# zenghjian/SceneSplat

Measured on AMD Instinct MI355X. Metric: Gaussians/s encoder fwd+bwd, 102k-pt chunks, higher is better.
Workload: dtype bf16

## Files before the change

### include/scenesplat_hip.h

```cpp
#ifndef SCENESPLAT_HIP_H
#define SCENESPLAT_HIP_H
#include <stddef.h>
#include <stdint.h>

#ifdef __cplusplus
extern "C" {
#endif

struct ihipStream_t;
typedef struct ihipStream_t* ss_stream_t;

#define SS_MAX_ORDERS 8
enum { SS_ORDER_Z = 0, SS_ORDER_Z_TRANS = 1, SS_ORDER_HILBERT = 2, SS_ORDER_HILBERT_TRANS = 3 };
enum { SS_DTYPE_F32 = 0, SS_DTYPE_BF16 = 1 };
enum { SS_ATTN_SIMT = 0, SS_ATTN_MFMA = 1 };

int ss_version(void);

int ss_serialize_encode(const int32_t* grid_coord, const int32_t* batch, int64_t n, int depth, const int* orders,
                        int num_orders, int64_t* codes, ss_stream_t stream);
int ss_offsets_to_batch(const int32_t* offsets, int num_batches, int64_t n, int32_t* batch, ss_stream_t stream);
int ss_count_duplicates(const int64_t* sorted_keys, int64_t n, int32_t* count, ss_stream_t stream);
int ss_grid_coord_max(const int32_t* grid_coord, int64_t n, int32_t* out_max, ss_stream_t stream);
size_t ss_argsort_workspace_bytes(int64_t n, int num_segments);
// ... 52 lines not shown
                      int num_heads, int sections, float sec0_scale, ss_stream_t stream);
int ss_window_attn_hm_fwd(const void* hm, const int32_t* sidx, const int32_t* win_start, int num_windows, int max_window,
                          int64_t n, int64_t n_pad, int channels, int num_heads, void* out, float* neg_lse2,
                          ss_stream_t stream);
size_t ss_window_attn_hm_bwd_workspace_bytes(int64_t n, int64_t n_pad, int channels, int num_heads);
int ss_window_attn_hm_bwd(const void* hm, const void* out, const void* dout, const float* neg_lse2, const int32_t* gidx,
                          const int32_t* sidx, const int32_t* win_start, int num_windows, int max_window, int64_t n,
                          int64_t n_pad, int channels, int num_heads, float scale, void* dqkv, void* workspace,
                          size_t workspace_bytes, ss_stream_t stream);

int ss_window_attn_rpe_fwd(const void* qkv, const int32_t* gidx, const int32_t* sidx, const int32_t* win_start,
                           int num_windows, int max_window, int64_t n, int64_t n_pad, int channels, int num_heads,
                           float scale, int dtype, int impl, const int32_t* grid_coord, const float* table, int pos_bnd,
                           void* out, float* lse, ss_stream_t stream);
size_t ss_window_attn_rpe_bwd_workspace_bytes(int64_t n, int64_t n_pad, int channels, int num_heads, int dtype,
                                              int num_windows, int max_window, int pos_bnd);
int ss_window_attn_rpe_bwd(const void* qkv, const void* out, const void* dout, const float* lse, const int32_t* gidx,
                           const int32_t* sidx, const int32_t* win_start, int num_windows, int max_window, int64_t n,
                           int64_t n_pad, int channels, int num_heads, float scale, int dtype, int impl,
                           const int32_t* grid_coord, const float* table, int pos_bnd, void* dqkv, float* dtable,
                           void* workspace, size_t workspace_bytes, ss_stream_t stream);

int ss_subm_rulebook(const int32_t* grid_coord, const int32_t* batch, int64_t n, int depth,
                     const int64_t* zkeys_sorted, const int32_t* zorder, int swap_xy, int kernel_size, int32_t* nbr,
                     ss_stream_t stream);
int ss_subm_tap_mask_keys(const int32_t* nbr, const int32_t* order, int64_t n, int taps, int coarse_bits, int64_t* keys,
                          ss_stream_t stream);
int64_t ss_subm_rulebook_table_size(int64_t n);
int ss_subm_rulebook_hashed(const int32_t* grid_coord, const int32_t* batch, int64_t n, int depth, int kernel_size, int32_t* nbr,
                            void* workspace, size_t workspace_bytes, ss_stream_t stream);

int ss_subm_conv_fwd(const void* in, const void* weight, const float* bias, const int32_t* nbr, const int32_t* rowperm,
                     void* out, int64_t n, int cin, int cout, int taps, int out_dtype, ss_stream_t stream);
int ss_subm_weight_mirror(const void* w, void* wt, int cout, int taps, int cin, ss_stream_t stream);
int ss_stream_create_cu_mask(int nwords, const uint32_t* mask, void** stream_out);
int ss_subm_im2col(const void* src, const int32_t* nbr, void* dst, int64_t n, int taps, int64_t row_bytes, ss_stream_t stream);
int ss_gemm8_ok(int64_t m, int k, int n, int taps);
int ss_subm_conv_fwd_pipe(const void* in, const void* weight, const float* bias, const int32_t* nbr, const int32_t* rowperm,
                          void* out, int64_t n, int cin, int cout, int taps, int out_dtype, ss_stream_t stream);
int ss_subm_conv_fwd_pipe_walk(const void* in, const void* weight, const float* bias, const int32_t* nbr_walk, const int32_t* rowperm,
                               void* out, int64_t n, int cin, int cout, int taps, int out_dtype, ss_stream_t stream);
int ss_subm_conv_fwd_uses_pipe(int64_t n, int cin, int cout, int taps);
int ss_subm_conv_fwd_walk(const void* in, const void* weight, const float* bias, const int32_t* nbr, const int32_t* nbr_walk,
                          const int32_t* rowperm, void* out, int64_t n, int cin, int cout, int taps, int out_dtype, ss_stream_t stream);
int ss_linear_fwd(const void* x, const void* weight, const float* bias, void* out, int64_t m, int k, int n, int out_dtype,
                  ss_stream_t stream);
int ss_wgrad_xcd_order(void);
int ss_wgrad_set_xcd_order(int on);
int ss_wgrad8_ok(int64_t n, int cin, int cout, int taps);
int ss_subm_conv_wgrad_pipe(const void* in, const void* dout, const int32_t* nbr, const int32_t* rowperm,
                            const int32_t* blk_count, const int32_t* blk_list, float* dweight, int64_t n, int cin, int cout,
                            int taps, ss_stream_t stream);
int ss_linear_wgrad(const void* x, const void* dy, float* dweight, float* dbias, int64_t m, int k_in, int n_out,
                    ss_stream_t stream);
int ss_linear_wgrad_group_plan(int64_t m, int k_in, int n_out, int64_t* desc_words);
int ss_linear_wgrad_tiles(int k_in, int n_out);
int ss_linear_wgrad_group_plan2(int64_t m, int k_in, int n_out, int launch_tiles, int64_t* desc_words);
int ss_linear_wgrad_group(const int64_t* desc, const int32_t* wg_start, int nprob, int total_workgroups, ss_stream_t stream);
int ss_subm_conv_splits(int64_t n, int cout, int taps);
int ss_subm_conv_fwd_splitk(const void* in, const void* weight, const float* bias, const int32_t* nbr, const int32_t* rowperm,
                            float* acc32, int64_t n, int cin, int cout, int taps, int splits, ss_stream_t stream);
int ss_subm_block_lists(const int32_t* nbr, const int32_t* rowperm, int64_t n, int taps, int32_t* blk_count,
                        int32_t* blk_list, ss_stream_t stream);
int ss_subm_conv_wgrad(const void* in, const void* dout, const int32_t* nbr, const int32_t* rowperm,
                       const int32_t* blk_count, const int32_t* blk_list, float* dweight, int64_t n, int cin, int cout,
                       int taps, ss_stream_t stream);

int ss_subm_f32_ok(int cin_padded, int cout);
int ss_subm_f32_fwd(const float* in, const float* wq, const float* bias, const int32_t* nbr_walk, const int32_t* rowperm,
                    float* out, int64_t n, int cin_padded, int cout, int taps, ss_stream_t stream);
int ss_subm_f32_dgrad_dup(const float* dout_folded, const float* wq, const int32_t* nbr_walk, const int32_t* rowperm, float* din,
                          int64_t n, int cin_padded, int cout, int taps, ss_stream_t stream);
int ss_subm_f32_wgrad(const float* in, const float* dout, const int32_t* nbr_walk, const int32_t* rowperm,
                      const int32_t* blk_count, const int32_t* blk_list, float* dweight, int64_t n, int cin_padded,
                      int cin, int cout, int taps, ss_stream_t stream);

int ss_subm_conv_wgrad_pipe_walk(const void* in, const void* dout, const int32_t* nbr_walk, const int32_t* rowperm,
                                 const int32_t* blk_count, const int32_t* blk_list, float* dweight, int64_t n, int cin, int cout,
                                 int taps, ss_stream_t stream);
int ss_subm_conv_wgrad_uses_pipe(int64_t n, int cin, int cout, int taps);
int ss_subm_conv_wgrad_walk(const void* in, const void* dout, const int32_t* nbr, const int32_t* nbr_walk, const int32_t* rowperm,
                            const int32_t* blk_count, const int32_t* blk_list, float* dweight, int64_t n, int cin, int cout,
                            int taps, ss_stream_t stream);

int ss_add_layernorm_fwd(const void* x, int x_dtype, const void* y, int y_dtype, const float* rowscale,
                         const float* gamma, const float* beta, float eps, void* xout, int xout_dtype, void* xcopy_bf16,
                         void* h, int h_dtype, float* mean, float* rstd, int64_t n, int channels, ss_stream_t stream);
int ss_ln_add_ln_fwd(const void* x, int x_dtype, const void* t, int t_dtype, const float* gamma0, const float* beta0, float eps0,
                     const float* gamma1, const float* beta1, float eps1, float* xout, void* h, int h_dtype, float* stats,
                     int64_t n, int channels, ss_stream_t stream);
int ss_ln_add_ln_bwd(const float* g_xout, const void* g_h, int g_h_dtype, const float* xout, const void* t, int t_dtype,
                     const float* stats, const float* gamma0, const float* gamma1, void* g_x, int g_x_dtype, void* g_t,
                     int g_t_dtype, float* part, int64_t n, int channels, int nblocks, ss_stream_t stream);
int ss_add_layernorm_bwd_blocks(int64_t n);

int ss_block_tail_rows(void);
int ss_block_tail_bwd_blocks(int64_t n);
int ss_block_tail_fwd(const void* feat, const float* x, const float* rs1, const float* rs2, const void* wp, const void* bp,
                      const void* w1, const void* b1, const void* w2, const void* b2, int bias_dtype, const float* gamma, const float* beta,
                      float eps, float* x_mid, float* mean, float* rstd, void* h2, void* u, void* a, float* x_out,
                      void* xcopy_bf16, int64_t n, int channels, ss_stream_t stream);
int ss_block_tail_bwd(const float* g_xout, const void* g_xcopy_bf16, const float* x_mid, const float* mean, const float* rstd,
                      const void* u, const float* rs1, const float* rs2, const float* gamma, const void* wp_t, const void* w1_t,
                      const void* w2_t, float* g_mid, void* dfeat, void* dy2, void* du, void* dy1, float* part, int64_t n,
                      int channels, int nblocks, ss_stream_t stream);
int ss_group_partial_sums_outputs_per_workgroup(void);
int ss_group_partial_sums(const int64_t* desc, const int32_t* wg_start, int nprob, int total_workgroups, ss_stream_t stream);
int ss_transpose16_group(const int64_t* desc, const int32_t* wg_start, int nprob, int total_workgroups, ss_stream_t stream);
int ss_subm_weight_mirror_group_tile(void);
int ss_subm_weight_mirror_group(const int64_t* desc, const int32_t* wg_start, int nprob, int total_workgroups, ss_stream_t stream);
int ss_add_layernorm_bwd(const void* g_xout, int g_xout_dtype, const void* g_xcopy, int g_xcopy_dtype, const void* g_h,
                         int g_h_dtype, const void* v, int v_dtype, const float* mean, const float* rstd,
                         const float* gamma, const float* rowscale, void* g_x, int g_x_dtype, void* g_y, int g_y_dtype,
                         float* dgamma_part, float* dbeta_part, int64_t n, int channels, int nblocks, ss_stream_t stream);

int ss_col_stats(const void* x, int x_dtype, float* shift_out, float* psum, float* psq, int64_t n, int channels,
                 int nblocks, ss_stream_t stream);
int ss_bn_stats_finish(const float* part, const float* shift, int nblocks, int channels, int64_t n, float momentum, float eps,
                       float* running_mean, float* running_var, int64_t* num_batches, float* mean, float* rstd,
                       ss_stream_t stream);
int ss_bn_bwd_finish(const float* part, int nblocks, int channels, int64_t n, float* sums, float* coef, ss_stream_t stream);
int ss_bn_act_fwd(const void* x, int x_dtype, const float* mean, const float* rstd, const float* gamma, const float* beta,
                  int act, void* y, int y_dtype, int64_t n, int channels, ss_stream_t stream);
int ss_bn_act_bwd_reduce(const void* dy, int dy_dtype, const void* x, int x_dtype, const float* mean, const float* rstd,
                         const float* gamma, const float* beta, int act, float* pdz, float* pdzx, int64_t n, int channels,
                         int nblocks, ss_stream_t stream);
int ss_bn_act_bwd_apply(const void* dy, int dy_dtype, const void* x, int x_dtype, const float* mean, const float* rstd,
                        const float* gamma, const float* beta, int act, const float* c1, const float* c2, void* dx,
                        int dx_dtype, int64_t n, int channels, ss_stream_t stream);

int ss_feat_text_scan(const void* feat_bf16, const void* text_bf16, int64_t n, int dim, int num_classes, float* max_prob,
                      int32_t* argmax, const int32_t* idx, float* pred_accum, ss_stream_t stream);

int ss_lang_head_blocks(int64_t n);
int ss_lang_head_fwd(const void* feat, int feat_dtype, const void* target, int target_dtype, const unsigned char* mask,
                     int normalize, void* p_out, int p_dtype, float* rowstat, float* part, float* sums, int64_t n,
                     int channels, ss_stream_t stream);
int ss_lang_head_bwd(const void* feat, int feat_dtype, const void* target, int target_dtype, const unsigned char* mask,
                     int normalize, const float* rowstat, const float* coef, const void* dp_extra, int dp_dtype,
                     void* dfeat, int dfeat_dtype, int64_t n, int channels, ss_stream_t stream);

size_t ss_seg_loss_workspace_bytes(int64_t n, int num_classes);
int ss_seg_loss_fwd(const void* logits, int dtype, const int64_t* labels, int64_t n, int num_classes, int64_t ignore_index,
                    const unsigned char* class_seen, int lovasz, float* rowstat, float* glov, int32_t* present, float* sums,
                    void* workspace, size_t workspace_bytes, ss_stream_t stream);
int ss_seg_loss_bwd(const void* logits, int dtype, const int64_t* labels, int64_t n, int num_classes, int64_t ignore_index,
                    const float* rowstat, const float* glov, const int32_t* present, const float* coef, void* dlogits,
                    ss_stream_t stream);
int ss_seg_iou(const void* logits, int dtype, const int32_t* pred, const int64_t* target, int64_t n, int num_classes,
               int64_t ignore_index, int64_t* out, ss_stream_t stream);

int ss_gather_rows(const void* src, const int32_t* idx, void* dst, int64_t n_dst, int64_t row_bytes, ss_stream_t stream);
int ss_scatter_rows(const void* src, const int32_t* idx, void* dst, int64_t n_src, int64_t row_bytes, ss_stream_t stream);
int ss_gather_add_rows(const void* a, const void* b, const int32_t* idx, void* dst, int64_t n, int channels, int dtype,
                       ss_stream_t stream);
int ss_dup_fold_rows(const void* src, const int64_t* sorted_keys, const int32_t* order, void* dst, int64_t n, int channels,
                     int dtype, ss_stream_t stream);
int ss_dup_zero_rows(const int64_t* sorted_keys, const int32_t* order, void* x, int64_t n, int64_t row_bytes, ss_stream_t stream);
int ss_segment_reduce(const void* src, const int32_t* indices, const int32_t* idx_ptr, void* out, int64_t n_seg,
                      int channels, int dtype, int mean, ss_stream_t stream);
int ss_segment_minmax(const void* src, const int32_t* indices, const int32_t* idx_ptr, void* out, int32_t* arg, int64_t n_seg,
                      int channels, int dtype, int is_max, ss_stream_t stream);
int ss_segment_minmax_bwd(const void* dout, const int32_t* arg, void* dsrc, int64_t n_seg, int channels, int dtype,
                          ss_stream_t stream);
int ss_segment_bcast(const void* dout, const int32_t* cluster, const int32_t* idx_ptr, void* dsrc, int64_t n,
                     int channels, int dtype, int mean, ss_stream_t stream);
// ... 97 lines not shown
```

### scenesplat_amd/_lib.py

```python
import ctypes
import os

import torch

_HERE = os.path.dirname(os.path.abspath(__file__))
LIB_PATH = os.path.join(_HERE, "lib", "libscenesplat_hip.so")

c_p = ctypes.c_void_p
c_i = ctypes.c_int
c_i64 = ctypes.c_int64
c_f = ctypes.c_float
c_sz = ctypes.c_size_t

PROTOTYPES = {
    "ss_version": (c_i, []),
    "ss_serialize_encode": (c_i, [c_p, c_p, c_i64, c_i, ctypes.POINTER(c_i), c_i, c_p, c_p]),
    "ss_offsets_to_batch": (c_i, [c_p, c_i, c_i64, c_p, c_p]),
    "ss_count_duplicates": (c_i, [c_p, c_i64, c_p, c_p]),
    "ss_grid_coord_max": (c_i, [c_p, c_i64, c_p, c_p]),
    "ss_argsort_workspace_bytes": (c_sz, [c_i64, c_i]),
    "ss_argsort_i64": (c_i, [c_p, c_i, c_i64, c_i, c_p, c_p, c_p, c_p, c_sz, c_p]),
    "ss_pool_partition_workspace_bytes": (c_sz, [c_i64]),
    "ss_pool_partition": (c_i, [c_p, c_p, c_i64, c_i, c_p, c_p, c_p, c_p, c_p, c_sz, c_p]),
    "ss_pool_level_attrs": (c_i, [c_p, c_i64, c_i64, c_p, c_p, c_p, c_i, c_i, c_p, c_p, c_p, c_p]),
    "ss_batch_offsets": (c_i, [c_p, c_p, c_i64, c_i, c_p, c_p]),
    "ss_window_index": (c_i, [c_p, c_p, c_p, c_i, c_i, c_i64, c_p, c_p, c_p]),
    "ss_window_attn_fwd": (c_i, [c_p, c_p, c_p, c_p, c_i, c_i, c_i64, c_i64, c_i, c_i, c_f, c_i, c_i, c_p, c_p, c_p]),
    "ss_window_attn_bwd_workspace_bytes": (c_sz, [c_i64, c_i64, c_i, c_i, c_i]),
    "ss_window_attn_bwd": (c_i, [c_p, c_p, c_p, c_p, c_p, c_p, c_p, c_i, c_i, c_i64, c_i64, c_i, c_i, c_f, c_i, c_i,
                                 c_p, c_p, c_sz, c_p]),
    "ss_window_attn_rpe_fwd": (c_i, [c_p, c_p, c_p, c_p, c_i, c_i, c_i64, c_i64, c_i, c_i, c_f, c_i, c_i, c_p, c_p, c_i,
                                     c_p, c_p, c_p]),
    "ss_window_attn_rpe_bwd_workspace_bytes": (c_sz, [c_i64, c_i64, c_i, c_i, c_i, c_i, c_i, c_i]),
    "ss_window_attn_rpe_bwd": (c_i, [c_p, c_p, c_p, c_p, c_p, c_p, c_p, c_i, c_i, c_i64, c_i64, c_i, c_i, c_f, c_i, c_i,
                                     c_p, c_p, c_i, c_p, c_p, c_p, c_sz, c_p]),
    "ss_gelu": (c_i, [c_p, c_p, c_p, c_i64, c_i, c_p]),
    "ss_row_keep_scales": (c_i, [c_p, c_p, c_p, c_i64, c_p]),
    "ss_stream_capture_status": (c_i, [c_p]),
    "ss_stream_capture_id": (ctypes.c_ulonglong, [c_p]),
    "ss_cast_bf16_group": (c_i, [c_p, c_p, c_i, c_i, c_p]),
    "ss_cast_bf16_group_elems_per_workgroup": (c_i, []),
    "ss_optim_group_elems_per_workgroup": (c_i, []),
    "ss_grad_sqnorm_group": (c_i, [c_p, c_p, c_i, c_i, c_p, c_p]),
    "ss_grad_norm_finish": (c_i, [c_p, c_i, c_f, c_p, c_p]),
    "ss_adamw_group": (c_i, [c_p, c_p, c_i, c_i, c_p, c_p]),
    "ss_pdnorm_channels_per_workgroup": (c_i, []),
    "ss_pdnorm_mod_fwd": (c_i, [c_p, c_p, c_i, c_i, c_p, c_i, c_i, c_p]),
    "ss_pdnorm_mod_bwd": (c_i, [c_p, c_p, c_i, c_i, c_p, c_i, c_i, c_i, c_p, c_p, c_p]),
    "ss_linear_fwd_headmajor": (c_i, [c_p, c_p, c_p, c_p, c_p, c_i64, c_i, c_i, c_i, c_i, c_f, c_p]),
    "ss_headmajor_pack": (c_i, [c_p, c_i, c_p, c_p, c_i64, c_i, c_i, c_i, c_f, c_p]),
    "ss_window_attn_hm_fwd": (c_i, [c_p, c_p, c_p, c_i, c_i, c_i64, c_i64, c_i, c_i, c_p, c_p, c_p]),
    "ss_window_attn_hm_bwd_workspace_bytes": (c_sz, [c_i64, c_i64, c_i, c_i]),
    "ss_window_attn_hm_bwd": (c_i, [c_p, c_p, c_p, c_p, c_p, c_p, c_p, c_i, c_i, c_i64, c_i64, c_i, c_i, c_f, c_p, c_p, c_sz, c_p]),
    "ss_subm_rulebook": (c_i, [c_p, c_p, c_i64, c_i, c_p, c_p, c_i, c_i, c_p, c_p]),
    "ss_subm_conv_fwd": (c_i, [c_p, c_p, c_p, c_p, c_p, c_p, c_i64, c_i, c_i, c_i, c_i, c_p]),
    "ss_stream_create_cu_mask": (c_i, [c_i, c_p, c_p]),
    "ss_ln_add_ln_fwd": (c_i, [c_p, c_i, c_p, c_i, c_p, c_p, c_f, c_p, c_p, c_f, c_p, c_p, c_i, c_p, c_i64, c_i, c_p]),
    "ss_ln_add_ln_bwd": (c_i, [c_p, c_p, c_i, c_p, c_p, c_i, c_p, c_p, c_p, c_p, c_i, c_p, c_i, c_p, c_i64, c_i, c_i, c_p]),
    "ss_segment_minmax": (c_i, [c_p, c_p, c_p, c_p, c_p, c_i64, c_i, c_i, c_i, c_p]),
    "ss_segment_minmax_bwd": (c_i, [c_p, c_p, c_p, c_i64, c_i, c_i, c_p]),
    "ss_subm_rulebook_table_size": (c_i64, [c_i64]),
    "ss_subm_rulebook_hashed": (c_i, [c_p, c_p, c_i64, c_i, c_i, c_p, c_p, ctypes.c_size_t, c_p]),
    "ss_subm_tap_mask_keys": (c_i, [c_p, c_p, c_i64, c_i, c_i, c_p, c_p]),
    "ss_subm_weight_mirror": (c_i, [c_p, c_p, c_i, c_i, c_i, c_p]),
    "ss_subm_im2col": (c_i, [c_p, c_p, c_p, c_i64, c_i, c_i64, c_p]),
    "ss_gemm8_ok": (c_i, [c_i64, c_i, c_i, c_i]),
    "ss_subm_conv_fwd_pipe": (c_i, [c_p, c_p, c_p, c_p, c_p, c_p, c_i64, c_i, c_i, c_i, c_i, c_p]),
    "ss_linear_fwd": (c_i, [c_p, c_p, c_p, c_p, c_i64, c_i, c_i, c_i, c_p]),
    "ss_wgrad_xcd_order": (c_i, []),
    "ss_wgrad_set_xcd_order": (c_i, [c_i]),
    "ss_wgrad8_ok": (c_i, [c_i64, c_i, c_i, c_i]),
    "ss_subm_conv_wgrad_pipe": (c_i, [c_p, c_p, c_p, c_p, c_p, c_p, c_p, c_i64, c_i, c_i, c_i, c_p]),
    "ss_linear_wgrad": (c_i, [c_p, c_p, c_p, c_p, c_i64, c_i, c_i, c_p]),
    "ss_linear_wgrad_group_plan": (c_i, [c_i64, c_i, c_i, c_p]),
    "ss_linear_wgrad_tiles": (c_i, [c_i, c_i]),
    "ss_linear_wgrad_group_plan2": (c_i, [c_i64, c_i, c_i, c_i, c_p]),
    "ss_linear_wgrad_group": (c_i, [c_p, c_p, c_i, c_i, c_p]),
    "ss_subm_conv_splits": (c_i, [c_i64, c_i, c_i]),
    "ss_subm_conv_fwd_splitk": (c_i, [c_p, c_p, c_p, c_p, c_p, c_p, c_i64, c_i, c_i, c_i, c_i, c_p]),
    "ss_subm_block_lists": (c_i, [c_p, c_p, c_i64, c_i, c_p, c_p, c_p]),
    "ss_subm_conv_wgrad": (c_i, [c_p, c_p, c_p, c_p, c_p, c_p, c_p, c_i64, c_i, c_i, c_i, c_p]),
    "ss_subm_conv_fwd_pipe_walk": (c_i, [c_p, c_p, c_p, c_p, c_p, c_p, c_i64, c_i, c_i, c_i, c_i, c_p]),
    "ss_subm_conv_fwd_uses_pipe": (c_i, [c_i64, c_i, c_i, c_i]),
    "ss_subm_conv_fwd_walk": (c_i, [c_p, c_p, c_p, c_p, c_p, c_p, c_p, c_i64, c_i, c_i, c_i, c_i, c_p]),
    "ss_subm_conv_wgrad_pipe_walk": (c_i, [c_p, c_p, c_p, c_p, c_p, c_p, c_p, c_i64, c_i, c_i, c_i, c_p]),
    "ss_subm_conv_wgrad_uses_pipe": (c_i, [c_i64, c_i, c_i, c_i]),
    "ss_subm_conv_wgrad_walk": (c_i, [c_p, c_p, c_p, c_p, c_p, c_p, c_p, c_p, c_i64, c_i, c_i, c_i, c_p]),
    "ss_subm_f32_ok": (c_i, [c_i, c_i]),
    "ss_subm_f32_fwd": (c_i, [c_p, c_p, c_p, c_p, c_p, c_p, c_i64, c_i, c_i, c_i, c_p]),
    "ss_subm_f32_dgrad_dup": (c_i, [c_p, c_p, c_p, c_p, c_p, c_i64, c_i, c_i, c_i, c_p]),
    "ss_dup_fold_rows": (c_i, [c_p, c_p, c_p, c_p, c_i64, c_i, c_i, c_p]),
    "ss_dup_zero_rows": (c_i, [c_p, c_p, c_p, c_i64, c_i64, c_p]),
    "ss_subm_f32_wgrad": (c_i, [c_p, c_p, c_p, c_p, c_p, c_p, c_p, c_i64, c_i, c_i, c_i, c_i, c_p]),
    "ss_add_layernorm_fwd": (c_i, [c_p, c_i, c_p, c_i, c_p, c_p, c_p, c_f, c_p, c_i, c_p, c_p, c_i, c_p, c_p, c_i64, c_i, c_p]),
    "ss_add_layernorm_bwd_blocks": (c_i, [c_i64]),
    "ss_block_tail_rows": (c_i, []),
    "ss_block_tail_bwd_blocks": (c_i, [c_i64]),
    "ss_block_tail_fwd": (c_i, [c_p] * 10 + [c_i, c_p, c_p, c_f] + [c_p] * 8 + [c_i64, c_i, c_p]),
    "ss_block_tail_bwd": (c_i, [c_p] * 18 + [c_i64, c_i, c_i, c_p]),
    "ss_group_partial_sums_outputs_per_workgroup": (c_i, []),
    "ss_group_partial_sums": (c_i, [c_p, c_p, c_i, c_i, c_p]),
    "ss_transpose16_group": (c_i, [c_p, c_p, c_i, c_i, c_p]),
    "ss_subm_weight_mirror_group_tile": (c_i, []),
    "ss_subm_weight_mirror_group": (c_i, [c_p, c_p, c_i, c_i, c_p]),
    "ss_add_layernorm_bwd": (c_i, [c_p, c_i, c_p, c_i, c_p, c_i, c_p, c_i, c_p, c_p, c_p, c_p, c_p, c_i, c_p, c_i, c_p, c_p,
                                   c_i64, c_i, c_i, c_p]),
    "ss_col_stats": (c_i, [c_p, c_i, c_p, c_p, c_p, c_i64, c_i, c_i, c_p]),
    "ss_bn_stats_finish": (c_i, [c_p, c_p, c_i, c_i, c_i64, c_f, c_f, c_p, c_p, c_p, c_p, c_p, c_p]),
    "ss_bn_bwd_finish": (c_i, [c_p, c_i, c_i, c_i64, c_p, c_p, c_p]),
    "ss_bn_act_fwd": (c_i, [c_p, c_i, c_p, c_p, c_p, c_p, c_i, c_p, c_i, c_i64, c_i, c_p]),
    "ss_bn_act_bwd_reduce": (c_i, [c_p, c_i, c_p, c_i, c_p, c_p, c_p, c_p, c_i, c_p, c_p, c_i64, c_i, c_i, c_p]),
    "ss_bn_act_bwd_apply": (c_i, [c_p, c_i, c_p, c_i, c_p, c_p, c_p, c_p, c_i, c_p, c_p, c_p, c_i, c_i64, c_i, c_p]),
    "ss_feat_text_scan": (c_i, [c_p, c_p, c_i64, c_i, c_i, c_p, c_p, c_p, c_p, c_p]),
    "ss_lang_head_blocks": (c_i, [c_i64]),
    "ss_lang_head_fwd": (c_i, [c_p, c_i, c_p, c_i, c_p, c_i, c_p, c_i, c_p, c_p, c_p, c_i64, c_i, c_p]),
    "ss_lang_head_bwd": (c_i, [c_p, c_i, c_p, c_i, c_p, c_i, c_p, c_p, c_p, c_i, c_p, c_i, c_i64, c_i, c_p]),
    "ss_seg_loss_workspace_bytes": (c_sz, [c_i64, c_i]),
    "ss_seg_loss_fwd": (c_i, [c_p, c_i, c_p, c_i64, c_i, c_i64, c_p, c_i, c_p, c_p, c_p, c_p, c_p, c_sz, c_p]),
    "ss_seg_loss_bwd": (c_i, [c_p, c_i, c_p, c_i64, c_i, c_i64, c_p, c_p, c_p, c_p, c_p, c_p]),
    "ss_seg_iou": (c_i, [c_p, c_i, c_p, c_p, c_i64, c_i, c_i64, c_p, c_p]),
    "ss_gather_rows": (c_i, [c_p, c_p, c_p, c_i64, c_i64, c_p]),
    "ss_scatter_rows": (c_i, [c_p, c_p, c_p, c_i64, c_i64, c_p]),
    "ss_gather_add_rows": (c_i, [c_p, c_p, c_p, c_p, c_i64, c_i, c_i, c_p]),
    "ss_segment_reduce": (c_i, [c_p, c_p, c_p, c_p, c_i64, c_i, c_i, c_i, c_p]),
    "ss_segment_bcast": (c_i, [c_p, c_p, c_p, c_p, c_i64, c_i, c_i, c_i, c_p]),
    "ss_aug_bbox_blocks": (c_i, [c_i64]),
    "ss_aug_bbox": (c_i, [c_p, c_i64, c_p, c_p, c_p, c_p]),
    "ss_aug_gaussians": (c_i, [c_p, c_p, c_p, c_p, c_i64, c_p, c_p, c_i, c_p, c_p, c_i, c_f, c_f, c_p, ctypes.c_uint64, c_p]),
    "ss_aug_elastic": (c_i, [c_p, c_i64, c_p, c_i, c_i, c_i, c_p, c_f, c_f, c_p]),
    "ss_aug_color": (c_i, [c_p, c_i64, c_i, c_p, c_p, c_f, c_p, c_f, c_p, ctypes.c_uint64, c_i, c_p]),
    "ss_voxel_pick_labelled": (c_i, [c_p, c_p, c_i64, c_p, c_i64, c_p, c_p]),
    "ss_color_chain_blocks": (c_i, [c_i64]),
    "ss_color_chain": (c_i, [c_p, c_i64, c_i, c_p, c_p, c_p, c_p, c_p]),
    "ss_voxel_blur_table_size": (c_i64, [c_i64]),
    "ss_voxel_blur_workspace_bytes": (c_sz, [c_i64]),
    "ss_voxel_blur": (c_i, [c_p, c_p, c_i64, c_p, c_p, c_p, c_p, c_p, c_i, c_f, c_p, c_sz, c_p]),
    "ss_mask_max_samples": (c_i, []),
    "ss_mask_key_bits": (c_i, []),
    "ss_mask_keys": (c_i, [c_p, c_p, c_i, c_i64, c_f, c_p, c_p, c_p]),
    "ss_mask_patches": (c_i, [c_p, c_p, c_p, c_i, c_i64, c_p, c_p, c_p, c_p, c_p]),
    "ss_mask_select_blocks": (c_i, [c_i64]),
    "ss_mask_select": (c_i, [c_p, c_p, c_p, c_p, c_i, c_i64, c_p, c_p, c_p, c_p, c_p, c_p, c_p]),
    "ss_mask_token_fwd": (c_i, [c_p, c_i, c_p, c_p, c_i64, c_i, c_p, c_p]),
    "ss_mask_token_bwd_blocks": (c_i, [c_i64]),
    "ss_mask_token_bwd_span": (c_i64, [c_i64]),
    "ss_mask_token_bwd": (c_i, [c_p, c_i, c_p, c_i64, c_i, c_p, c_p, c_p, c_p]),
    "ss_ema_group": (c_i, [c_p, c_p, c_i, c_i, c_f, c_f, c_p]),
    "ss_knn_grid_table_size": (c_i64, [c_i64]),
    "ss_knn_grid_workspace_bytes": (c_sz, [c_i64]),
    "ss_knn_grid_keys": (c_i, [c_p, c_p, c_i, c_i64, c_f, c_f, c_f, c_f, c_p, c_p]),
    "ss_knn_grid_build": (c_i, [c_p, c_p, c_p, c_i64, c_p, c_sz, c_p, c_p]),
    "ss_knn_grid_query": (c_i, [c_i, c_i, c_p, c_p, c_p, c_p, c_i, c_f, c_f, c_f, c_f, c_i, c_i, c_i, c_i64, c_p, c_p, c_p, c_p]),
    "ss_ball_grid_query": (c_i, [c_i, c_i, c_f, c_f, c_p, c_p, c_p, c_p, c_p, c_i, c_f, c_f, c_f, c_f, c_i, c_i, c_i, c_i64, c_p, c_p, c_p, c_p]),
    "ss_knn_query": (c_i, [c_i, c_i, c_p, c_p, c_p, c_p, c_i, c_p, c_p, c_p]),
    "ss_ball_query_workspace_bytes": (c_sz, [c_i]),
    "ss_ball_query": (c_i, [c_i, c_i, c_f, c_f, c_p, c_p, c_p, c_p, c_i, c_p, c_p, c_p, c_sz, c_p]),
    "ss_random_ball_query": (c_i, [c_i, c_i, c_f, c_f, c_p, c_p, c_p, c_p, c_p, c_i, c_p, c_p, c_p]),
    "ss_farthest_point_sampling": (c_i, [c_i, c_p, c_p, c_p, c_p, c_p, c_p]),
    "ss_grouping_fwd": (c_i, [c_i, c_i, c_i, c_p, c_p, c_p, c_p]),
    "ss_grouping_bwd": (c_i, [c_i, c_i, c_i, c_p, c_p, c_p, c_p]),
    "ss_subtraction_fwd": (c_i, [c_i, c_i, c_i, c_p, c_p, c_p, c_p, c_p]),
    "ss_subtraction_bwd": (c_i, [c_i, c_i, c_i, c_p, c_p, c_p, c_p, c_p]),
    "ss_aggregation_fwd": (c_i, [c_i, c_i, c_i, c_i, c_p, c_p, c_p, c_p, c_p, c_p]),
    "ss_aggregation_bwd": (c_i, [c_i, c_i, c_i, c_i, c_p, c_p, c_p, c_p, c_p, c_p, c_p, c_p, c_p]),
    "ss_interpolation_fwd": (c_i, [c_i, c_i, c_i, c_p, c_p, c_p, c_p, c_p]),
    "ss_interpolation_bwd": (c_i, [c_i, c_i, c_i, c_p, c_p, c_p, c_p, c_p]),
    "ss_attention_relation_fwd": (c_i, [c_i, c_i, c_i, c_p, c_p, c_p, c_p, c_p, c_p, c_p]),
    "ss_attention_relation_bwd": (c_i, [c_i, c_i, c_i, c_p, c_p, c_p, c_p, c_p, c_p, c_p, c_p, c_p, c_p]),
    "ss_attention_fusion_fwd": (c_i, [c_i, c_i, c_i, c_p, c_p, c_p, c_p, c_p, c_p]),
    "ss_attention_fusion_bwd": (c_i, [c_i, c_i, c_i, c_p, c_p, c_p, c_p, c_p, c_p, c_p, c_p]),
# ... 44 lines not shown
```

### scenesplat_amd/csrc/subm_conv.hip

```cpp
#include "common.h"
#include "../../include/scenesplat_hip.h"
#include <stdlib.h>

typedef __attribute__((ext_vector_type(8))) __bf16 bf8_t;
typedef __attribute__((ext_vector_type(4))) short s4_t;
typedef __attribute__((ext_vector_type(8))) short s8_t;
typedef __attribute__((address_space(3))) s4_t lds_s4_t;
#define MFMA16(a, b, c) __builtin_amdgcn_mfma_f32_16x16x32_bf16((a), (b), (c), 0, 0, 0)

#define CV_THREADS 256
#define CV_BM 128
#define CV_BN 128
#define CV_BK 64
#ifndef SS_CONV_BIG_MIN_TILES
#define SS_CONV_BIG_MIN_TILES 64
#endif
#ifndef SS_CONV_DMA_SMALL
#define SS_CONV_DMA_SMALL false
#endif
#ifndef SS_CONV_DMA_BIG
#define SS_CONV_DMA_BIG false
#endif
#define CV_TG 27

// ... 145 lines not shown
        for (int mi = 0; mi < TM; ++mi)
#pragma unroll
          for (int ni = 0; ni < TN; ++ni) acc[mi][ni] = MFMA16(bf[ni], af[mi], acc[mi][ni]);
      }
      if (!DMA && it + 1 < iters) stage_write(b ^ 1);
      __syncthreads();
    }
  }
#pragma unroll
  for (int mi = 0; mi < TM; ++mi) {
    const int row = rowid_s[16 * TM * wm + 16 * mi + lq];
    if (row < 0) continue;
#pragma unroll
    for (int ni = 0; ni < TN; ++ni) {
      const int col = n0 + 16 * TN * wn + 16 * ni + 4 * g;
      if (acc32) {
#pragma unroll
        for (int r = 0; r < 4; ++r)
          if (col + r < Cout) atomicAdd(acc32 + (int64_t)row * Cout + col + r, acc[mi][ni][r] + ((bias && blockIdx.z == 0) ? bias[col + r] : 0.f));
      } else if (col + 3 < Cout && (Cout & 3) == 0) {
        float4 v = make_float4(acc[mi][ni][0], acc[mi][ni][1], acc[mi][ni][2], acc[mi][ni][3]);
        if (bias) { float4 bv = *reinterpret_cast<const float4*>(bias + col); v.x += bv.x; v.y += bv.y; v.z += bv.z; v.w += bv.w; }
        OutT* op = out + (int64_t)row * Cout + col;
        if (sizeof(OutT) == 2) {
          uint2 u; u.x = pack_bf16x2(v.x, v.y); u.y = pack_bf16x2(v.z, v.w);
          *reinterpret_cast<uint2*>(op) = u;
        } else {
          *reinterpret_cast<float4*>(op) = v;
        }
      } else {
#pragma unroll
        for (int r = 0; r < 4; ++r)
          if (col + r < Cout) ElemIO<OutT>::store(out + (int64_t)row * Cout + col + r, acc[mi][ni][r] + (bias ? bias[col + r] : 0.f));
      }
    }
  }
}

__global__ void k_subm_block_flags(const int32_t* __restrict__ nbr, const int32_t* __restrict__ rowperm, int n, int nblocks,
                                   int32_t* __restrict__ blk_list) {
  const int t = blockIdx.y, wave = threadIdx.x >> 6, lane = threadIdx.x & 63;
  const int blk = blockIdx.x * 4 + wave;
  if (blk >= nblocks) return;
  const int k = blk * 64 + lane;
  int j = -1;
  if (k < n) j = nbr[(int64_t)t * n + (rowperm ? rowperm[k] : k)];
  unsigned long long m = __ballot(j >= 0);
  if (lane == 0) blk_list[(int64_t)t * nblocks + blk] = m != 0ULL;
}

__global__ void __launch_bounds__(1024) k_subm_block_compact(int nblocks, int32_t* __restrict__ blk_count,
                                                              int32_t* __restrict__ blk_list) {
  __shared__ int wsum[16];
  __shared__ int base_s;
  int32_t* row = blk_list + (int64_t)blockIdx.x * nblocks;
  const int tid = threadIdx.x, wave = tid >> 6, lane = tid & 63;
  if (tid == 0) base_s = 0;
  __syncthreads();
  for (int c0 = 0; c0 < nblocks; c0 += 1024) {
    const int b = c0 + tid;
    const int f = b < nblocks ? row[b] : 0;
    unsigned long long m = __ballot(f != 0);
    if (lane == 0) wsum[wave] = __popcll(m);
    __syncthreads();
    int before = base_s;
    for (int w = 0; w < wave; ++w) before += wsum[w];
    if (f) row[before + __popcll(m & ((1ULL << lane) - 1ULL))] = b;
    __syncthreads();
    if (tid == 0) { int s = 0; for (int w = 0; w < 16; ++w) s += wsum[w]; base_s += s; }
    __syncthreads();
  }
  if (tid == 0) blk_count[blockIdx.x] = base_s;
}

extern "C" int ss_subm_block_lists(const int32_t* nbr, const int32_t* rowperm, int64_t n, int taps, int32_t* blk_count,
                                   int32_t* blk_list, hipStream_t stream) {
  if (n <= 0 || taps <= 0 || n >= (1LL << 31)) return SS_ERR_ARG;
  const int nblocks = ss_div_up(n, 64);
  SS_LAUNCH(k_subm_block_flags, dim3(ss_div_up(nblocks, 4), taps), dim3(256), 0, stream, nbr, rowperm, (int)n, nblocks, blk_list);
  SS_LAUNCH(k_subm_block_compact, dim3(taps), dim3(1024), 0, stream, nblocks, blk_count, blk_list);
  return SS_OK;
}

template <int WM, int WN, int TM, int TN>
__global__ void __launch_bounds__(64 * WM * WN)
k_subm_wgrad(const unsigned short* __restrict__ in, const unsigned short* __restrict__ dout,
             const int32_t* __restrict__ nbr, const int32_t* __restrict__ rowperm, const int32_t* __restrict__ blk_count,
             const int32_t* __restrict__ blk_list, float* __restrict__ dW, int n, int Cin, int Cout, int taps, int ntiles_n,
             int nblocks_total) {
  constexpr int THREADS = 64 * WM * WN, BMc = 16 * TM * WM, BNc = 16 * TN * WN;
  constexpr int ARB = BMc * 2, BRB = BNc * 2;
  constexpr int AIMG = 64 * ARB, BIMG = 64 * BRB;
  constexpr int ACH = BMc / 8, BCH = BNc / 8;
  constexpr int NLA = (64 * ACH) / THREADS, NLB = (64 * BCH) / THREADS;
  __shared__ __attribute__((aligned(16))) char smem[2 * (AIMG + BIMG)];
  __shared__ int32_t isite_s[2][64], jsite_s[2][64];
  const int tid = threadIdx.x, wave = tid >> 6, lane = tid & 63, lq = lane & 15, g = lane >> 4;
  const int wm = wave / WN, wn = wave % WN;
  const int m0 = (blockIdx.x / ntiles_n) * BMc, n0 = (blockIdx.x % ntiles_n) * BNc;
  const int tap = blockIdx.y;
  const int cnt = blk_count[tap];
  const int per = (cnt + gridDim.z - 1) / gridDim.z;
  const int beg = blockIdx.z * per, end = min(cnt, beg + per);
  const int nblk = end - beg;
  if (nblk <= 0) return;
  const int32_t* list = blk_list + (int64_t)tap * nblocks_total + beg;
  auto img_off = [](int row, int ch, int rb) { return row * rb + ((((ch & 15) ^ ((row & 7) << 1)) | (ch & ~15)) << 4); };
  f32x4_t acc[TM][TN];
#pragma unroll
  for (int mi = 0; mi < TM; ++mi)
#pragma unroll
    for (int ni = 0; ni < TN; ++ni) acc[mi][ni] = f32x4_t{0.f, 0.f, 0.f, 0.f};
  uint4 sa[NLA], sb[NLB];
  auto index_load = [&](int b, int blk) {
    if (tid < 64) {
      int k = list[blk] * 64 + tid;
      int i = k < n ? (rowperm ? rowperm[k] : k) : -1;
      isite_s[b][tid] = i;
      jsite_s[b][tid] = i >= 0 ? nbr[(int64_t)tap * n + i] : -1;
    }
  };
  auto stage_load = [&](int b) {
#pragma unroll
    for (int i = 0; i < NLA; ++i) {
      int c = i * THREADS + tid;
      int r = c / ACH, co = m0 + (c % ACH) * 8;
      uint4 v = make_uint4(0, 0, 0, 0);
      if (jsite_s[b][r] >= 0 && co < Cout) v = *reinterpret_cast<const uint4*>(dout + (int64_t)isite_s[b][r] * Cout + co);
      sa[i] = v;
    }
#pragma unroll
    for (int i = 0; i < NLB; ++i) {
      int c = i * THREADS + tid;
      int r = c / BCH, ci = n0 + (c % BCH) * 8;
      uint4 v = make_uint4(0, 0, 0, 0);
      int sj = jsite_s[b][r];
      if (sj >= 0 && ci < Cin) v = *reinterpret_cast<const uint4*>(in + (int64_t)sj * Cin + ci);
      sb[i] = v;
    }
  };
  auto stage_write = [&](int b) {
    char* A = smem + b * (AIMG + BIMG); char* B = A + AIMG;
#pragma unroll
    for (int i = 0; i < NLA; ++i) { int c = i * THREADS + tid; *reinterpret_cast<uint4*>(A + img_off(c / ACH, c % ACH, ARB)) = sa[i]; }
#pragma unroll
    for (int i = 0; i < NLB; ++i) { int c = i * THREADS + tid; *reinterpret_cast<uint4*>(B + img_off(c / BCH, c % BCH, BRB)) = sb[i]; }
  };
  index_load(0, 0);
  __syncthreads();
  stage_load(0); stage_write(0);
  if (nblk > 1) index_load(1, 1);
  __syncthreads();
  for (int blk = 0; blk < nblk; ++blk) {
    const int b = blk & 1;
    const bool have_next = blk + 1 < nblk;
    if (have_next) stage_load(b ^ 1);
    {
      const char* A = smem + b * (AIMG + BIMG); const char* B = A + AIMG;
#pragma unroll
      for (int kk = 0; kk < 2; ++kk) {
        bf8_t af[TM], bf[TN];
        const int r0 = 32 * kk + 4 * g + (lq >> 2);
#pragma unroll
        for (int mi = 0; mi < TM; ++mi) {
          int ch = (16 * TM * wm + 16 * mi) / 8 + ((lq & 3) >> 1);
          af[mi] = cv_cat(cv_lds_tr(A + img_off(r0, ch, ARB) + 8 * (lq & 1)), cv_lds_tr(A + img_off(r0 + 16, ch, ARB) + 8 * (lq & 1)));
        }
#pragma unroll
        for (int ni = 0; ni < TN; ++ni) {
          int ch = (16 * TN * wn + 16 * ni) / 8 + ((lq & 3) >> 1);
          bf[ni] = cv_cat(cv_lds_tr(B + img_off(r0, ch, BRB) + 8 * (lq & 1)), cv_lds_tr(B + img_off(r0 + 16, ch, BRB) + 8 * (lq & 1)));
        }
#pragma unroll
        for (int mi = 0; mi < TM; ++mi)
#pragma unroll
          for (int ni = 0; ni < TN; ++ni) acc[mi][ni] = MFMA16(af[mi], bf[ni], acc[mi][ni]);
      }
    }
    __syncthreads();
    if (have_next) stage_write(b ^ 1);
    if (blk + 2 < nblk) index_load(b, blk + 2);
    __syncthreads();
  }
#pragma unroll
  for (int mi = 0; mi < TM; ++mi)
#pragma unroll
    for (int r = 0; r < 4; ++r) {
      int co = m0 + 16 * TM * wm + 16 * mi + 4 * g + r;
      if (co < Cout) {
#pragma unroll
        for (int ni = 0; ni < TN; ++ni) {
          int ci = n0 + 16 * TN * wn + 16 * ni + lq;
          if (ci < Cin) atomicAdd(dW + ((int64_t)co * taps + tap) * Cin + ci, acc[mi][ni][r]);
        }
      }
    }
}

template <typename OutT>
static int subm_gemm_launch(const unsigned short* x, const unsigned short* w, const float* bias, const int32_t* nbr,
                            const int32_t* rowperm, OutT* out, int n, int cin, int cout, int taps, hipStream_t stream,
                            float* acc32 = nullptr, int splits = 1) {
  if (acc32) {
    dim3 g(ss_div_up(n, 128), ss_div_up(cout, 128), splits), b(256);
    SS_LAUNCH((k_subm_gemm<OutT, 2, 2, 4, 4, SS_CONV_DMA_SMALL>), g, b, 0, stream, x, w, bias, nbr, rowperm, out, n, cin, cout, taps, acc32);
    return SS_OK;
  }
  if (cout >= 256 && (int64_t)ss_div_up(n, 256) * ss_div_up(cout, 256) >= SS_CONV_BIG_MIN_TILES) {
    dim3 g(ss_div_up(n, 256), ss_div_up(cout, 256)), b(512);
    SS_LAUNCH((k_subm_gemm<OutT, 4, 2, 4, 8, SS_CONV_DMA_BIG>), g, b, 0, stream, x, w, bias, nbr, rowperm, out, n, cin, cout, taps, (float*)nullptr);
  } else {
    dim3 g(ss_div_up(n, 128), ss_div_up(cout, 128)), b(256);
    SS_LAUNCH((k_subm_gemm<OutT, 2, 2, 4, 4, SS_CONV_DMA_SMALL>), g, b, 0, stream, x, w, bias, nbr, rowperm, out, n, cin, cout, taps, (float*)nullptr);
  }
  return SS_OK;
}

static int conv_pipe_mode() {
  static int mode = -2;
  if (mode == -2) { const char* e = getenv("SS_CONV_PIPE"); mode = e ? atoi(e) : -1; }
  return mode;
}

extern "C" int ss_subm_conv_fwd(const void* in, const void* weight, const float* bias, const int32_t* nbr,
                                const int32_t* rowperm, void* out, int64_t n, int cin, int cout, int taps, int out_dtype,
                                hipStream_t stream) {
  if (n < 0 || cin <= 0 || cout <= 0 || taps <= 0 || (cin & 7) || n >= (1LL << 31)) return SS_ERR_ARG;
  if (n == 0) return SS_OK;
  if (ss_gemm8_ok(n, cin, cout, taps) && conv_pipe_mode() != 0 &&
      (conv_pipe_mode() == 1 || (cout >= 256 && (int64_t)ss_div_up(n, 256) * ss_div_up(cout, 256) >= SS_CONV_BIG_MIN_TILES)))
    return ss_subm_conv_fwd_pipe(in, weight, bias, nbr, rowperm, out, n, cin, cout, taps, out_dtype, stream);
  const unsigned short* x = (const unsigned short*)in; const unsigned short* w = (const unsigned short*)weight;
  if (out_dtype == SS_BF16) return subm_gemm_launch<unsigned short>(x, w, bias, nbr, rowperm, (unsigned short*)out, (int)n, cin, cout, taps, stream);
  if (out_dtype == SS_F32) return subm_gemm_launch<float>(x, w, bias, nbr, rowperm, (float*)out, (int)n, cin, cout, taps, stream);
  return SS_ERR_ARG;
}

static bool conv_fwd_uses_pipe(int64_t n, int cin, int cout, int taps) {
  return ss_gemm8_ok(n, cin, cout, taps) && conv_pipe_mode() != 0 &&
         (conv_pipe_mode() == 1 || (cout >= 256 && (int64_t)ss_div_up(n, 256) * ss_div_up(cout, 256) >= SS_CONV_BIG_MIN_TILES));
}
extern "C" int ss_subm_conv_fwd_uses_pipe(int64_t n, int cin, int cout, int taps) { return conv_fwd_uses_pipe(n, cin, cout, taps) ? 1 : 0; }

extern "C" int ss_subm_conv_fwd_walk(const void* in, const void* weight, const float* bias, const int32_t* nbr,
                                     const int32_t* nbr_walk, const int32_t* rowperm, void* out, int64_t n, int cin, int cout,
                                     int taps, int out_dtype, hipStream_t stream) {
  if (n < 0 || cin <= 0 || cout <= 0 || taps <= 0 || (cin & 7) || n >= (1LL << 31)) return SS_ERR_ARG;
  if (n == 0) return SS_OK;
  if (nbr_walk && conv_fwd_uses_pipe(n, cin, cout, taps))
    return ss_subm_conv_fwd_pipe_walk(in, weight, bias, nbr_walk, rowperm, out, n, cin, cout, taps, out_dtype, stream);
  return ss_subm_conv_fwd(in, weight, bias, nbr, rowperm, out, n, cin, cout, taps, out_dtype, stream);
}

extern "C" int ss_subm_conv_splits(int64_t n, int cout, int taps) {
  int64_t tiles = (int64_t)ss_div_up(n, 128) * ss_div_up(cout, 128);
  if (tiles >= 192) return 1;
  int z = (int)((256 + tiles - 1) / tiles);
  if (z > taps) z = taps;
  if (z > 9) z = 9;
  return z < 2 ? 1 : z;
}
extern "C" int ss_subm_conv_fwd_splitk(const void* in, const void* weight, const float* bias, const int32_t* nbr,
                                       const int32_t* rowperm, float* acc32, int64_t n, int cin, int cout, int taps,
                                       int splits, hipStream_t stream) {
  if (n < 0 || cin <= 0 || cout <= 0 || taps <= 0 || (cin & 7) || n >= (1LL << 31) || splits < 1 || !acc32) return SS_ERR_ARG;
  if (n == 0) return SS_OK;
  return subm_gemm_launch<float>((const unsigned short*)in, (const unsigned short*)weight, bias, nbr, rowperm, acc32,
                                 (int)n, cin, cout, taps, stream, acc32, splits);
}

static bool conv_wgrad_uses_pipe(int64_t n, int cin, int cout, int taps) {
  static int mode = -2;
  if (mode == -2) { const char* e = getenv("SS_WGRAD_PIPE"); mode = e ? atoi(e) : -1; }
  return mode != 0 && ss_wgrad8_ok(n, cin, cout, taps) && (mode == 1 || (cout >= 128 && cin >= 128));
}
extern "C" int ss_subm_conv_wgrad_uses_pipe(int64_t n, int cin, int cout, int taps) { return conv_wgrad_uses_pipe(n, cin, cout, taps) ? 1 : 0; }

extern "C" int ss_subm_conv_wgrad_walk(const void* in, const void* dout, const int32_t* nbr, const int32_t* nbr_walk,
                                       const int32_t* rowperm, const int32_t* blk_count, const int32_t* blk_list, float* dweight,
                                       int64_t n, int cin, int cout, int taps, hipStream_t stream);

extern "C" int ss_subm_conv_wgrad(const void* in, const void* dout, const int32_t* nbr, const int32_t* rowperm,
                                  const int32_t* blk_count, const int32_t* blk_list, float* dweight, int64_t n, int cin,
                                  int cout, int taps, hipStream_t stream) {
  return ss_subm_conv_wgrad_walk(in, dout, nbr, nullptr, rowperm, blk_count, blk_list, dweight, n, cin, cout, taps, stream);
}

extern "C" int ss_subm_conv_wgrad_walk(const void* in, const void* dout, const int32_t* nbr, const int32_t* nbr_walk,
                                       const int32_t* rowperm, const int32_t* blk_count, const int32_t* blk_list, float* dweight,
                                       int64_t n, int cin, int cout, int taps, hipStream_t stream) {
  if (n < 0 || cin <= 0 || cout <= 0 || taps <= 0 || (cin & 7) || (cout & 7) || n >= (1LL << 31)) return SS_ERR_ARG;
  if (n == 0) return SS_OK;
  if (conv_wgrad_uses_pipe(n, cin, cout, taps)) {
    if (nbr_walk) return ss_subm_conv_wgrad_pipe_walk(in, dout, nbr_walk, rowperm, blk_count, blk_list, dweight, n, cin, cout, taps, stream);
    return ss_subm_conv_wgrad_pipe(in, dout, nbr, rowperm, blk_count, blk_list, dweight, n, cin, cout, taps, stream);
  }
  const int nblocks = ss_div_up(n, 64);
  const bool big = cout >= 256 && cin >= 256 && nblocks >= 1024;
  const int T = big ? 256 : 128;
  const int tm = ss_div_up(cout, T), tn = ss_div_up(cin, T);
  int splits = (big ? 3072 : 6144) / (tm * tn * taps);
  if (splits > nblocks / 8) splits = nblocks / 8;
  if (splits < 1) splits = 1;
  dim3 g(tm * tn, taps, splits);
  const unsigned short* x = (const unsigned short*)in; const unsigned short* go = (const unsigned short*)dout;
  if (big)
    SS_LAUNCH((k_subm_wgrad<2, 4, 8, 4>), g, dim3(512), 0, stream, x, go, nbr, rowperm, blk_count, blk_list, dweight, (int)n, cin, cout, taps, tn, nblocks);
  else
    SS_LAUNCH((k_subm_wgrad<2, 2, 4, 4>), g, dim3(256), 0, stream, x, go, nbr, rowperm, blk_count, blk_list, dweight, (int)n, cin, cout, taps, tn, nblocks);
  return SS_OK;
}
```

### scenesplat_amd/csrc/subm_f32.hip

```cpp
#include "common.h"
#include "../../include/scenesplat_hip.h"

#define F32MFMA(a, b, c) __builtin_amdgcn_mfma_f32_32x32x2f32((a), (b), (c), 0, 0, 0)
#define SF_TG 32

__device__ __forceinline__ float4 sf_row_or_zero(const float* __restrict__ base, int row, int width, int col) {
  float4 v = *reinterpret_cast<const float4*>(base + (int64_t)max(row, 0) * width + col);
  const bool ok = row >= 0;
  v.x = ok ? v.x : 0.f; v.y = ok ? v.y : 0.f; v.z = ok ? v.z : 0.f; v.w = ok ? v.w : 0.f;
  return v;
}

template <int CI>
__global__ void __launch_bounds__(256) __attribute__((amdgpu_waves_per_eu(3, 3)))
k_subm_f32_fwd(const float* __restrict__ in, const float* __restrict__ wq, const float* __restrict__ bias,
               const int32_t* __restrict__ nbr_walk, const int32_t* __restrict__ rowperm, float* __restrict__ out, int n, int taps,
               int winner_tap) {
  constexpr int NCH = CI / 4;
  constexpr int NQ = CI / 8;
  constexpr int NA = (32 * NCH) / 64;
  constexpr int PL = 32 * 16 + 16;
  __shared__ __attribute__((aligned(16))) char smem[4 * (NCH * PL + SF_TG * 32 * 4)];
  const int tid = threadIdx.x, wave = tid >> 6, lane = tid & 63, i = lane & 31, kk = lane >> 5;
  char* const aimg = smem + wave * (NCH * PL + SF_TG * 32 * 4);
  int32_t* const nb_s = reinterpret_cast<int32_t*>(aimg + NCH * PL);
  const int m0 = (blockIdx.x * 4 + wave) * 32;
  if (m0 >= n) return;
  const int site = (m0 + i < n) ? (rowperm ? rowperm[m0 + i] : m0 + i) : -1;
  const int keep = (winner_tap < 0 || site < 0) ? 1 : (nbr_walk[(int64_t)winner_tap * n + m0 + i] == site ? 1 : 0);
  f32x16_t acc;
#pragma unroll
  for (int r = 0; r < 16; ++r) acc[r] = 0.f;
  for (int tg = 0; tg < taps; tg += SF_TG) {
    const int nt = min(SF_TG, taps - tg);
    int nbv[SF_TG / 2];
#pragma unroll
    for (int u = 0; u < SF_TG / 2; ++u) {
      const int tt = 2 * u + kk;
      const int v = nbr_walk[(int64_t)(tg + min(tt, nt - 1)) * n + min(m0 + i, n - 1)];
      nbv[u] = (tt < nt && site >= 0) ? v : -1;
    }
    unsigned mask = 0u;
#pragma unroll
    for (int u = 0; u < SF_TG / 2; ++u) {
      nb_s[(2 * u + kk) * 32 + i] = nbv[u];
      const unsigned long long b = __ballot(nbv[u] >= 0);
      mask |= ((unsigned)(b & 0xffffffffULL) != 0u ? 1u : 0u) << (2 * u);
      mask |= ((unsigned)(b >> 32) != 0u ? 1u : 0u) << (2 * u + 1);
    }
    mask = __builtin_amdgcn_readfirstlane(mask);
    auto issue = [&](int t, float4 (&ra)[NA], float4 (&rb)[NQ]) {
#pragma unroll
      for (int r = 0; r < NA; ++r) {
        const int e = r * 64 + lane, si = e / NCH, c = e - si * NCH;
        const int nb = nb_s[t * 32 + si];
        ra[r] = sf_row_or_zero(in, nb, CI, c * 4);
      }
#pragma unroll
      for (int q = 0; q < NQ; ++q) rb[q] = *reinterpret_cast<const float4*>(wq + ((((int64_t)(tg + t) * NQ + q) * 2 + kk) * 32 + i) * 4);
    };
    auto consume = [&](const float4 (&ra)[NA], const float4 (&rb)[NQ]) {
#pragma unroll
      for (int r = 0; r < NA; ++r) {
        const int e = r * 64 + lane, si = e / NCH, c = e - si * NCH;
        *reinterpret_cast<float4*>(aimg + c * PL + si * 16) = ra[r];
      }
#pragma unroll
      for (int q = 0; q < NQ; ++q) {
        const float4 a = *reinterpret_cast<const float4*>(aimg + (2 * q + kk) * PL + i * 16);
        acc = F32MFMA(a.x, rb[q].x, acc); acc = F32MFMA(a.y, rb[q].y, acc);
        acc = F32MFMA(a.z, rb[q].z, acc); acc = F32MFMA(a.w, rb[q].w, acc);
      }
    };
    if (mask) {
      float4 ra0[NA], rb0[NQ], ra1[NA], rb1[NQ];
      int t = __builtin_ctz(mask); mask &= mask - 1u;
      issue(t, ra0, rb0);
      while (true) {
        if (!mask) { consume(ra0, rb0); break; }
        t = __builtin_ctz(mask); mask &= mask - 1u;
        issue(t, ra1, rb1); consume(ra0, rb0);
        if (!mask) { consume(ra1, rb1); break; }
        t = __builtin_ctz(mask); mask &= mask - 1u;
        issue(t, ra0, rb0); consume(ra1, rb1);
      }
    }
  }
  const float bj = bias ? bias[i] : 0.f;
#pragma unroll
  for (int r = 0; r < 16; ++r) {
    const int row = (r & 3) + 8 * (r >> 2) + 4 * kk;
    const int s = __shfl(site, row, 64);
    const int kp = __shfl(keep, row, 64);
    if (s >= 0) out[(int64_t)s * 32 + i] = kp ? acc[r] + bj : 0.f;
  }
}

#define SF_WPER 4

template <int CI>
__global__ void __launch_bounds__(256) __attribute__((amdgpu_waves_per_eu(3, 3)))
k_subm_f32_wgrad(const float* __restrict__ in, const float* __restrict__ g, const int32_t* __restrict__ nbr_walk,
                 const int32_t* __restrict__ rowperm, const int32_t* __restrict__ blk_count, const int32_t* __restrict__ blk_list,
                 float* __restrict__ dW, int n, int taps, int cin, int nblocks) {
  constexpr int NCH = CI / 4;
  constexpr int NX = (32 * NCH) / 64;
  constexpr int WAVE_LDS = 2 * SF_WPER * 64 * 4 + 32 * 128 + 32 * CI * 4;
  __shared__ __attribute__((aligned(16))) char smem[4 * WAVE_LDS];
  const int tid = threadIdx.x, wave = tid >> 6, lane = tid & 63, j = lane & 31, kk = lane >> 5;
  int32_t* const site_s = reinterpret_cast<int32_t*>(smem + wave * WAVE_LDS);
  int32_t* const nb_s = site_s + SF_WPER * 64;
  char* const gimg = reinterpret_cast<char*>(nb_s + SF_WPER * 64);
  char* const ximg = gimg + 32 * 128;
  const int tap = blockIdx.y, share = blockIdx.x * 4 + wave;
  const int cnt = blk_count[tap];
  const int beg = share * SF_WPER, end = min(cnt, beg + SF_WPER);
  if (beg >= end) return;
  const int32_t* list = blk_list + (int64_t)tap * nblocks;
#pragma unroll
  for (int r = 0; r < SF_WPER; ++r) {
    const int b = beg + r;
    int site = -1, nb = -1;
    if (b < end) {
      const int k = list[b] * 64 + lane;
      if (k < n) { site = rowperm ? rowperm[k] : k; nb = nbr_walk[(int64_t)tap * n + k]; }
    }
    site_s[r * 64 + lane] = nb >= 0 ? site : -1;
    nb_s[r * 64 + lane] = nb;
  }
  const int nsub = (end - beg) * 2;
  auto issue = [&](int sb, float4 (&rg)[4], float4 (&rx)[NX]) {
#pragma unroll
    for (int r = 0; r < 4; ++r) {
      const int e = r * 64 + lane, si = e >> 3, c = e & 7;
      const int s2 = site_s[sb * 32 + si];
      rg[r] = sf_row_or_zero(g, s2, 32, c * 4);
    }
#pragma unroll
    for (int r = 0; r < NX; ++r) {
      const int e = r * 64 + lane, si = e / NCH, c = e - si * NCH;
      const int n2 = nb_s[sb * 32 + si];
      rx[r] = sf_row_or_zero(in, n2, CI, c * 4);
    }
  };
  f32x16_t acc;
#pragma unroll
  for (int r = 0; r < 16; ++r) acc[r] = 0.f;
  auto consume = [&](const float4 (&rg)[4], const float4 (&rx)[NX]) {
#pragma unroll
    for (int r = 0; r < 4; ++r) {
      const int e = r * 64 + lane;
      *reinterpret_cast<float4*>(gimg + (e >> 3) * 128 + (e & 7) * 16) = rg[r];
    }
#pragma unroll
    for (int r = 0; r < NX; ++r) {
      const int e = r * 64 + lane, si = e / NCH, c = e - si * NCH;
      *reinterpret_cast<float4*>(ximg + si * (CI * 4) + c * 16) = rx[r];
    }
#pragma unroll
    for (int u = 0; u < 16; ++u) {
      const float a = *reinterpret_cast<const float*>(gimg + (2 * u + kk) * 128 + j * 4);
      const float x = *reinterpret_cast<const float*>(ximg + (2 * u + kk) * (CI * 4) + (j & (CI - 1)) * 4);
      acc = F32MFMA(a, x, acc);
    }
  };
  {
    float4 rg0[4], rx0[NX], rg1[4], rx1[NX];
    int sb = 0;
    issue(0, rg0, rx0);
    while (true) {
      if (++sb >= nsub) { consume(rg0, rx0); break; }
      issue(sb, rg1, rx1); consume(rg0, rx0);
      if (++sb >= nsub) { consume(rg1, rx1); break; }
      issue(sb, rg0, rx0); consume(rg1, rx1);
    }
  }
  if (j < cin) {
#pragma unroll
    for (int r = 0; r < 16; ++r) {
      const int co = (r & 3) + 8 * (r >> 2) + 4 * kk;
      atomicAdd(dW + ((int64_t)co * taps + tap) * cin + j, acc[r]);
    }
  }
}

extern "C" int ss_subm_f32_ok(int cin_padded, int cout) { return cout == 32 && (cin_padded == 16 || cin_padded == 32); }

static int subm_f32_launch(const float* in, const float* wq, const float* bias, const int32_t* nbr_walk, const int32_t* rowperm,
                           float* out, int64_t n, int cin_padded, int cout, int taps, int winner_tap, hipStream_t stream) {
  if (n < 0 || n >= (1LL << 31) || taps <= 0 || !ss_subm_f32_ok(cin_padded, cout)) return SS_ERR_ARG;
  if (n == 0) return SS_OK;
  dim3 g(ss_div_up(n, 128)), b(256);
  if (cin_padded == 16) SS_LAUNCH((k_subm_f32_fwd<16>), g, b, 0, stream, in, wq, bias, nbr_walk, rowperm, out, (int)n, taps, winner_tap);
  else SS_LAUNCH((k_subm_f32_fwd<32>), g, b, 0, stream, in, wq, bias, nbr_walk, rowperm, out, (int)n, taps, winner_tap);
  return SS_OK;
}

extern "C" int ss_subm_f32_fwd(const float* in, const float* wq, const float* bias, const int32_t* nbr_walk, const int32_t* rowperm,
                               float* out, int64_t n, int cin_padded, int cout, int taps, hipStream_t stream) {
  return subm_f32_launch(in, wq, bias, nbr_walk, rowperm, out, n, cin_padded, cout, taps, -1, stream);
}

extern "C" int ss_subm_f32_dgrad_dup(const float* dout_folded, const float* wq, const int32_t* nbr_walk, const int32_t* rowperm,
                                     float* din, int64_t n, int cin_padded, int cout, int taps, hipStream_t stream) {
  if (!(taps & 1)) return SS_ERR_ARG;
  return subm_f32_launch(dout_folded, wq, nullptr, nbr_walk, rowperm, din, n, cin_padded, cout, taps, taps / 2, stream);
}

extern "C" int ss_subm_f32_wgrad(const float* in, const float* gout, const int32_t* nbr_walk, const int32_t* rowperm,
                                 const int32_t* blk_count, const int32_t* blk_list, float* dweight, int64_t n, int cin_padded,
                                 int cin, int cout, int taps, hipStream_t stream) {
  if (n < 0 || n >= (1LL << 31) || taps <= 0 || !ss_subm_f32_ok(cin_padded, cout) || cin <= 0 || cin > cin_padded) return SS_ERR_ARG;
  if (n == 0) return SS_OK;
  const int nblocks = ss_div_up(n, 64);
  dim3 g(ss_div_up(ss_div_up(nblocks, SF_WPER), 4), taps), b(256);
  if (cin_padded == 16)
    SS_LAUNCH((k_subm_f32_wgrad<16>), g, b, 0, stream, in, gout, nbr_walk, rowperm, blk_count, blk_list, dweight, (int)n, taps, cin, nblocks);
  else
    SS_LAUNCH((k_subm_f32_wgrad<32>), g, b, 0, stream, in, gout, nbr_walk, rowperm, blk_count, blk_list, dweight, (int)n, taps, cin, nblocks);
  return SS_OK;
}
```

### scenesplat_amd/csrc/wgrad8.hip

```cpp
#include "grouped.h"
#include "../../include/scenesplat_hip.h"
#include <stdlib.h>

typedef __attribute__((ext_vector_type(8))) __bf16 w8_bf8_t;
typedef __attribute__((ext_vector_type(4))) short w8_s4_t;
typedef __attribute__((ext_vector_type(8))) short w8_s8_t;
typedef __attribute__((address_space(3))) w8_s4_t w8_lds_s4_t;
#define W8_MFMA(a, b, c) __builtin_amdgcn_mfma_f32_16x16x32_bf16((a), (b), (c), 0, 0, 0)

#define W8_BUF 65536
#define W8_HALF 16384
#define W8_OFF_B 32768
#define W8_CHUNK 60
#define W8_OFF_ISITE 131072
#define W8_OFF_JSITE (W8_OFF_ISITE + W8_CHUNK * 64 * 4)
#define W8_LDS_BYTES (W8_OFF_JSITE + W8_CHUNK * 64 * 4)
#define W8_ZERO_ELEMS 4096

__device__ uint4 w8_zero[W8_ZERO_ELEMS / 8];

__device__ __forceinline__ void w8_glds16(const void* gsrc, unsigned lds_wave_base) {
  asm volatile("s_mov_b32 m0, %1\n\ts_nop 0\n\tglobal_load_lds_dwordx4 %0, off" ::"v"(gsrc), "s"(lds_wave_base) : "memory");
}
__device__ __forceinline__ w8_bf8_t w8_tr2(const char* p) {
  w8_s4_t lo = __builtin_amdgcn_ds_read_tr16_b64_v4i16((w8_lds_s4_t*)(p));
  w8_s4_t hi = __builtin_amdgcn_ds_read_tr16_b64_v4i16((w8_lds_s4_t*)(p + 16 * 256));
  w8_s8_t v = {lo[0], lo[1], lo[2], lo[3], hi[0], hi[1], hi[2], hi[3]};
  return __builtin_bit_cast(w8_bf8_t, v);
}

template <bool GATHER>
__device__ __forceinline__ void
w8_body(const unsigned short* __restrict__ X, const unsigned short* __restrict__ DY, const int32_t* __restrict__ nbr,
        const int32_t* __restrict__ rowperm, const int32_t* __restrict__ blk_count, const int32_t* __restrict__ blk_list,
        float* __restrict__ dW, float* __restrict__ dbias, int n, int Cin, int Cout, int taps, int ntn, int nblocks_total,
        int min_per, int ntiles, int nshares, const int L, const int walk = 0) {
  __shared__ __attribute__((aligned(16))) char smem[GATHER ? W8_LDS_BYTES : 2 * W8_BUF];
  int32_t* isite_s = reinterpret_cast<int32_t*>(smem + W8_OFF_ISITE);
  int32_t* jsite_s = reinterpret_cast<int32_t*>(smem + W8_OFF_JSITE);
  const int tid = threadIdx.x, wave = tid >> 6, lane = tid & 63, lq = lane & 15, g = lane >> 4;
  const int wr = wave >> 2, wc = wave & 3;
  const int tile = L % ntiles, group = L / ntiles;
  const int tap = group % taps, share = group / taps;
  const int m0 = (tile / ntn) * 256, n0 = (tile % ntn) * 256;
  const int cnt = GATHER ? blk_count[tap] : nblocks_total;
  const int per = max((cnt + nshares - 1) / nshares, min_per);
  const int beg = share * per, end = min(cnt, beg + per);
  if (end <= beg) return;
  const int32_t* list = GATHER ? blk_list + (int64_t)tap * nblocks_total : nullptr;

  f32x4_t acc[2][4][2][2];
#pragma unroll
  for (int a = 0; a < 2; ++a)
#pragma unroll
    for (int mi = 0; mi < 4; ++mi)
#pragma unroll
      for (int b = 0; b < 2; ++b)
#pragma unroll
        for (int ni = 0; ni < 2; ++ni) acc[a][mi][b][ni] = f32x4_t{0.f, 0.f, 0.f, 0.f};

  const bool do_bias = !GATHER && dbias != nullptr && (tile % ntn) == 0;
  f32x4_t accb[2] = {f32x4_t{0.f, 0.f, 0.f, 0.f}, f32x4_t{0.f, 0.f, 0.f, 0.f}};
  w8_bf8_t ones;
  {
    w8_s8_t o = {0x3F80, 0x3F80, 0x3F80, 0x3F80, 0x3F80, 0x3F80, 0x3F80, 0x3F80};
    ones = __builtin_bit_cast(w8_bf8_t, o);
  }

  const int srow = wave * 4 + (lane >> 4);
  const int ssw = ((srow & 7) << 1);
  const int lch = (lane & 15) ^ ssw;
  int colA[2], colB[2];
#pragma unroll
  for (int h = 0; h < 2; ++h) {
    colA[h] = min(m0 + (lch >> 3) * 128 + h * 64 + (lch & 7) * 8, Cout - 8);
    colB[h] = min(n0 + (lch >> 2) * 64 + h * 32 + (lch & 3) * 8, Cin - 8);
  }
  const unsigned short* const zrow = reinterpret_cast<const unsigned short*>(w8_zero);
  const unsigned short* pA[2];
  const unsigned short* pB[2];
  int chunk_beg = beg, T = 0, staged = 0;
  int nis[2] = {-1, -1}, njs[2] = {-1, -1};
  auto prefetch_idx = [&]() {
    if (!GATHER || staged + 1 >= T) return;
#pragma unroll
    for (int j = 0; j < 2; ++j) {
      nis[j] = isite_s[(staged + 1) * 64 + srow + 32 * j];
      njs[j] = jsite_s[(staged + 1) * 64 + srow + 32 * j];
    }
  };
  auto make_rows = [&](int s) {
#pragma unroll
    for (int j = 0; j < 2; ++j) {
      if (GATHER) {
        pA[j] = njs[j] >= 0 ? DY + (int64_t)nis[j] * Cout : zrow;
        pB[j] = njs[j] >= 0 ? X + (int64_t)njs[j] * Cin : zrow;
      } else {
        int64_t k = (int64_t)(chunk_beg + s) * 64 + srow + 32 * j;
        pA[j] = k < n ? DY + k * Cout : zrow;
        pB[j] = k < n ? X + k * Cin : zrow;
      }
    }
  };
  auto advance = [&]() {
    if (staged + 1 >= T) return;
    ++staged;
    make_rows(staged);
  };
  const unsigned dst0 = __builtin_amdgcn_readfirstlane(
      (unsigned)(size_t)((__attribute__((address_space(3))) char*)smem) + (unsigned)wave * 1024u);
  auto stageA = [&](int buf, int h) {
    unsigned d = dst0 + buf * W8_BUF + h * W8_HALF;
    w8_glds16(pA[0] + colA[h], d);
    w8_glds16(pA[1] + colA[h], d + 8192);
  };
  auto stageB = [&](int buf, int h) {
    unsigned d = dst0 + buf * W8_BUF + W8_OFF_B + h * W8_HALF;
    w8_glds16(pB[0] + colB[h], d);
    w8_glds16(pB[1] + colB[h], d + 8192);
  };

  const int rsw = ((4 * (g & 1) + (lq >> 2)) << 1);
  const int rbase = (4 * g + (lq >> 2)) * 256 + 8 * (lq & 1);
  int oA[4], oB[2];
#pragma unroll
  for (int mi = 0; mi < 4; ++mi) oA[mi] = rbase + (((wr * 8 + 2 * mi + ((lq & 3) >> 1)) ^ rsw) << 4);
#pragma unroll
  for (int ni = 0; ni < 2; ++ni) oB[ni] = W8_OFF_B + rbase + (((wc * 4 + 2 * ni + ((lq & 3) >> 1)) ^ rsw) << 4);
  w8_bf8_t af[4][2], b0f[2][2], b1f[2][2];
  auto readA = [&](int buf, int h) {
    const char* base = smem + buf * W8_BUF + h * W8_HALF;
#pragma unroll
    for (int mi = 0; mi < 4; ++mi) {
      af[mi][0] = w8_tr2(base + oA[mi]);
      af[mi][1] = w8_tr2(base + oA[mi] + 32 * 256);
    }
  };
  auto readB = [&](int buf, int h, w8_bf8_t (&bf)[2][2]) {
    const char* base = smem + buf * W8_BUF + h * W8_HALF;
#pragma unroll
    for (int ni = 0; ni < 2; ++ni) {
      bf[ni][0] = w8_tr2(base + oB[ni]);
      bf[ni][1] = w8_tr2(base + oB[ni] + 32 * 256);
    }
  };
#define W8_MM(HA, HB, BF)                                                                         \
  _Pragma("unroll") for (int ks = 0; ks < 2; ++ks)                                                \
  _Pragma("unroll") for (int mi = 0; mi < 4; ++mi)                                                \
  _Pragma("unroll") for (int ni = 0; ni < 2; ++ni)                                                \
      acc[HA][mi][HB][ni] = W8_MFMA(af[mi][ks], BF[ni][ks], acc[HA][mi][HB][ni]);
#define W8_BIAS(HA)                                                                               \
  if (do_bias) {                                                                                  \
    if (wc == 0) { accb[HA] = W8_MFMA(af[0][0], ones, accb[HA]); accb[HA] = W8_MFMA(af[0][1], ones, accb[HA]); }       \
    else if (wc == 1) { accb[HA] = W8_MFMA(af[1][0], ones, accb[HA]); accb[HA] = W8_MFMA(af[1][1], ones, accb[HA]); }  \
    else if (wc == 2) { accb[HA] = W8_MFMA(af[2][0], ones, accb[HA]); accb[HA] = W8_MFMA(af[2][1], ones, accb[HA]); }  \
    else { accb[HA] = W8_MFMA(af[3][0], ones, accb[HA]); accb[HA] = W8_MFMA(af[3][1], ones, accb[HA]); }              \
  }
#define W8_BAR() do { __builtin_amdgcn_sched_barrier(0); __builtin_amdgcn_s_barrier(); __builtin_amdgcn_sched_barrier(0); } while (0)
#define W8_COMPUTE_BEGIN() do { W8_BAR(); asm volatile("s_waitcnt lgkmcnt(0)" ::: "memory"); __builtin_amdgcn_sched_barrier(0); __builtin_amdgcn_s_setprio(1); } while (0)
#define W8_COMPUTE_END() do { __builtin_amdgcn_s_setprio(0); W8_BAR(); } while (0)

  for (; chunk_beg < end; chunk_beg += (GATHER ? W8_CHUNK : (1 << 30))) {
    T = GATHER ? min(W8_CHUNK, end - chunk_beg) : end - chunk_beg;
    if (GATHER) {
      __syncthreads();
      if (walk) {
        constexpr int NH = 4;
        for (int e0 = 0; e0 < T * 64; e0 += NH * 512) {
          int kk[NH], is_[NH], js_[NH];
          const int laste = T * 64 - 1;
#pragma unroll
          for (int it = 0; it < NH; ++it) {
            const int e = min(e0 + it * 512 + tid, laste);
            kk[it] = list[chunk_beg + (e >> 6)] * 64 + (e & 63);
          }
#pragma unroll
          for (int it = 0; it < NH; ++it) {
            const int kc = min(kk[it], n - 1);
            is_[it] = rowperm ? rowperm[kc] : kc;
            js_[it] = nbr[(int64_t)tap * n + kc];
          }
#pragma unroll
          for (int it = 0; it < NH; ++it) {
            const int e = e0 + it * 512 + tid;
            if (e <= laste) {
              const bool ok = kk[it] < n;
              isite_s[e] = ok ? is_[it] : -1;
              jsite_s[e] = ok ? js_[it] : -1;
            }
          }
        }
      } else {
        for (int e = tid; e < T * 64; e += 512) {
          int k = list[chunk_beg + (e >> 6)] * 64 + (e & 63);
          int is = k < n ? (rowperm ? rowperm[k] : k) : -1;
          isite_s[e] = is;
          jsite_s[e] = is >= 0 ? nbr[(int64_t)tap * n + is] : -1;
        }
      }
      __syncthreads();
    }
    staged = -1;
    prefetch_idx();
    staged = 0;
    make_rows(0);
    prefetch_idx();
    stageB(0, 0); stageA(0, 0); stageB(0, 1); stageA(0, 1);
    advance();
    prefetch_idx();
    stageB(1, 0); stageA(1, 0); stageB(1, 1);
    asm volatile("s_waitcnt vmcnt(6)" ::: "memory");
    W8_BAR();
    if (wr == 1) W8_BAR();
    for (int t = 0; t < T; ++t) {
      const int buf = t & 1;
      readB(buf, 0, b0f);
      __builtin_amdgcn_sched_barrier(0);
      readA(buf, 0);
      stageA(buf ^ 1, 1);
      __builtin_amdgcn_sched_barrier(0);
      asm volatile("s_waitcnt lgkmcnt(15)" ::: "memory");
      W8_COMPUTE_BEGIN();
      W8_MM(0, 0, b0f)
      W8_COMPUTE_END();
      advance();
      readB(buf, 1, b1f);
      stageB(buf, 0);
      W8_COMPUTE_BEGIN();
      W8_MM(0, 1, b1f)
      W8_BIAS(0)
      W8_COMPUTE_END();
      readA(buf, 1);
      stageA(buf, 0);
      W8_COMPUTE_BEGIN();
      W8_MM(1, 1, b1f)
      W8_COMPUTE_END();
      stageB(buf, 1);
      prefetch_idx();
      asm volatile("s_waitcnt vmcnt(6)" ::: "memory");
      W8_COMPUTE_BEGIN();
      W8_MM(1, 0, b0f)
      W8_BIAS(1)
      W8_COMPUTE_END();
    }
    if (wr == 0) W8_BAR();
    asm volatile("s_waitcnt vmcnt(0)" ::: "memory");
  }

#pragma unroll
  for (int ha = 0; ha < 2; ++ha)
#pragma unroll
    for (int mi = 0; mi < 4; ++mi)
#pragma unroll
      for (int r = 0; r < 4; ++r) {
        const int co = m0 + 128 * wr + 64 * ha + 16 * mi + 4 * g + r;
        if (co >= Cout) continue;
        float* rowp = dW + ((int64_t)co * taps + tap) * Cin;
#pragma unroll
        for (int hb = 0; hb < 2; ++hb)
#pragma unroll
          for (int ni = 0; ni < 2; ++ni) {
            const int ci = n0 + 64 * wc + 32 * hb + 16 * ni + lq;
            if (ci < Cin) atomicAdd(rowp + ci, acc[ha][mi][hb][ni][r]);
          }
      }
  if (do_bias && lq == 0) {
#pragma unroll
    for (int ha = 0; ha < 2; ++ha)
#pragma unroll
      for (int r = 0; r < 4; ++r) {
        const int co = m0 + 128 * wr + 64 * ha + 16 * wc + 4 * g + r;
        if (co < Cout) atomicAdd(dbias + co, accb[ha][r]);
      }
  }
}

#undef W8_BIAS

#define W8_XG 3
__device__ __forceinline__ int w8_xcd_order(int L, int nb) {
  const int row = 8 * W8_XG, full = nb / row * row;
  if (L >= full) return L;
  const int xcd = L & 7, slot = L >> 3;
  return ((slot / W8_XG) * 8 + xcd) * W8_XG + slot % W8_XG;
}

template <bool GATHER>
__global__ void __launch_bounds__(512)
k_wgrad8(const unsigned short* __restrict__ X, const unsigned short* __restrict__ DY, const int32_t* __restrict__ nbr,
         const int32_t* __restrict__ rowperm, const int32_t* __restrict__ blk_count, const int32_t* __restrict__ blk_list,
         float* __restrict__ dW, float* __restrict__ dbias, int n, int Cin, int Cout, int taps, int ntn, int nblocks_total,
         int min_per, int ntiles, int nshares, int walk) {
  int L = (int)blockIdx.x;
  if (walk & 2) L = w8_xcd_order(L, (int)gridDim.x);
  w8_body<GATHER>(X, DY, nbr, rowperm, blk_count, blk_list, dW, dbias, n, Cin, Cout, taps, ntn, nblocks_total, min_per, ntiles,
                  nshares, L, walk & 1);
}

__global__ void __launch_bounds__(512)
k_wgrad8_group(const int64_t* __restrict__ desc, const int32_t* __restrict__ wg_start, int nprob, int nprob_flags) {
  const int b = blockIdx.x;
  const int p = group_owner(wg_start, nprob, b);
  const int64_t* d = desc + (int64_t)p * 8;
  const int64_t m = d[4];
  const uint64_t w5 = (uint64_t)d[5], w6 = (uint64_t)d[6], w7 = (uint64_t)d[7];
  const int k_in = (int)(w5 & 0xffffffffu), n_out = (int)(w5 >> 32);
  const int ntn = (int)(w6 & 0xffffffffu), ntiles = (int)(w6 >> 32);
  const int nshares = (int)(w7 & 0xffffffffu), min_per = (int)(w7 >> 32);
  int L = b - wg_start[p];
  if (nprob_flags & 1) {
    const int a = (8 - (wg_start[p] & 7)) & 7;
    if (L >= a) L = a + w8_xcd_order(L - a, nshares * ntiles - a);
  }
  w8_body<false>((const unsigned short*)d[0], (const unsigned short*)d[1], nullptr, nullptr, nullptr, nullptr, (float*)d[2],
                 (float*)d[3], (int)m, k_in, n_out, 1, ntn, (int)((m + 63) / 64), min_per, ntiles, nshares, L);
}

static int w8_xcd_flag = -1;
extern "C" int ss_wgrad_xcd_order(void) {
  if (w8_xcd_flag < 0) { const char* e = getenv("SS_WGRAD_XCD_TRIPLE"); w8_xcd_flag = (e && atoi(e) == 1) ? 1 : 0; }
  return w8_xcd_flag;
}
extern "C" int ss_wgrad_set_xcd_order(int on) { w8_xcd_flag = on ? 1 : 0; return SS_OK; }

extern "C" int ss_wgrad8_ok(int64_t n, int cin, int cout, int taps) {
  return n > 0 && n < (1LL << 31) && cin >= 8 && (cin & 7) == 0 && cin <= W8_ZERO_ELEMS && cout >= 8 && (cout & 7) == 0 &&
         cout <= W8_ZERO_ELEMS && taps >= 1;
}

static int w8_min_per(int64_t busy_tiles, int64_t est_blocks) {
  int64_t per = busy_tiles * est_blocks / 200;
  if (per < 8) per = 8;
  if (per > 160) per = 160;
  return (int)per;
}

static int w8_conv_launch(const void* in, const void* dout, const int32_t* nbr, const int32_t* rowperm, const int32_t* blk_count,
                          const int32_t* blk_list, float* dweight, int64_t n, int cin, int cout, int taps, int walk, hipStream_t stream);

extern "C" int ss_subm_conv_wgrad_pipe(const void* in, const void* dout, const int32_t* nbr, const int32_t* rowperm,
                                       const int32_t* blk_count, const int32_t* blk_list, float* dweight, int64_t n,
                                       int cin, int cout, int taps, hipStream_t stream) {
  return w8_conv_launch(in, dout, nbr, rowperm, blk_count, blk_list, dweight, n, cin, cout, taps, 0, stream);
}
extern "C" int ss_subm_conv_wgrad_pipe_walk(const void* in, const void* dout, const int32_t* nbr_walk, const int32_t* rowperm,
                                            const int32_t* blk_count, const int32_t* blk_list, float* dweight, int64_t n,
                                            int cin, int cout, int taps, hipStream_t stream) {
  return w8_conv_launch(in, dout, nbr_walk, rowperm, blk_count, blk_list, dweight, n, cin, cout, taps, 1, stream);
}

static int w8_conv_launch(const void* in, const void* dout, const int32_t* nbr, const int32_t* rowperm, const int32_t* blk_count,
                          const int32_t* blk_list, float* dweight, int64_t n, int cin, int cout, int taps, int walk, hipStream_t stream) {
  if (n == 0) return SS_OK;
  if (!ss_wgrad8_ok(n, cin, cout, taps) || !blk_count || !blk_list || !nbr) return SS_ERR_ARG;
  const int nblocks = ss_div_up(n, 64);
  const int tm = ss_div_up(cout, 256), tn = ss_div_up(cin, 256);
  static int env_per = -2;
  if (env_per == -2) { const char* e = getenv("SS_WGRAD_MINPER"); env_per = e ? atoi(e) : -1; }
  int min_per = env_per > 0 ? env_per : w8_min_per((int64_t)tm * tn * ((taps + 2) / 3), (int64_t)nblocks * 7 / 10);
  int splits = ss_div_up(nblocks, min_per);
  if (ss_wgrad_xcd_order()) walk |= 2;
  dim3 g((unsigned)((int64_t)taps * splits * tm * tn));
  SS_LAUNCH((k_wgrad8<true>), g, dim3(512), 0, stream, (const unsigned short*)in, (const unsigned short*)dout, nbr, rowperm,
            blk_count, blk_list, dweight, (float*)nullptr, (int)n, cin, cout, taps, tn, nblocks, min_per, tm * tn, splits, walk);
  return SS_OK;
}

static void w8_linear_plan(int64_t m, int k_in, int n_out, int* tm_, int* tn_, int* min_per_, int* splits_, int launch_tiles = 0) {
  const int nblocks = ss_div_up(m, 64);
  const int tm = ss_div_up(n_out, 256), tn = ss_div_up(k_in, 256);
  static int env_per = -2;
  if (env_per == -2) { const char* e = getenv("SS_WGRAD_MINPER"); env_per = e ? atoi(e) : -1; }
  static const int cus = [] {
    int dev = 0, n = 256;
    if (hipGetDevice(&dev) == hipSuccess) (void)hipDeviceGetAttribute(&n, hipDeviceAttributeMultiprocessorCount, dev);
    return n > 0 ? n : 256;
  }();
  const int tiles_all = launch_tiles > tm * tn ? launch_tiles : tm * tn;
  const int shares = cus / tiles_all > 0 ? cus / tiles_all : 1;
  int min_per = env_per > 0 ? env_per : (int)((nblocks + shares - 1) / shares);
  if (env_per <= 0 && min_per < 8) min_per = 8;
  if (min_per > nblocks) min_per = nblocks;
  *tm_ = tm; *tn_ = tn; *min_per_ = min_per; *splits_ = ss_div_up(nblocks, min_per);
}

extern "C" int ss_linear_wgrad_tiles(int k_in, int n_out) { return ss_div_up(n_out, 256) * ss_div_up(k_in, 256); }
extern "C" int ss_linear_wgrad_group_plan2(int64_t m, int k_in, int n_out, int launch_tiles, int64_t* desc_words) {
  if (m <= 0 || !ss_wgrad8_ok(m, k_in, n_out, 1) || !desc_words) return 0;
  int tm, tn, min_per, splits;
  w8_linear_plan(m, k_in, n_out, &tm, &tn, &min_per, &splits, launch_tiles);
  desc_words[5] = (int64_t)((uint64_t)(uint32_t)k_in | ((uint64_t)(uint32_t)n_out << 32));
  desc_words[6] = (int64_t)((uint64_t)(uint32_t)tn | ((uint64_t)(uint32_t)(tm * tn) << 32));
  desc_words[7] = (int64_t)((uint64_t)(uint32_t)splits | ((uint64_t)(uint32_t)min_per << 32));
  return splits * tm * tn;
}
extern "C" int ss_linear_wgrad_group_plan(int64_t m, int k_in, int n_out, int64_t* desc_words) {
  return ss_linear_wgrad_group_plan2(m, k_in, n_out, 0, desc_words);
}

extern "C" int ss_linear_wgrad_group(const int64_t* desc, const int32_t* wg_start, int nprob, int total_workgroups,
                                     hipStream_t stream) {
  SS_GROUP_GUARD(desc, wg_start, nprob, total_workgroups);
  if (nprob > 128) return SS_ERR_ARG;
  SS_LAUNCH(k_wgrad8_group, dim3((unsigned)total_workgroups), dim3(512), 0, stream, desc, wg_start, nprob, 0);
  return SS_OK;
}

extern "C" int ss_linear_wgrad(const void* x, const void* dy, float* dweight, float* dbias, int64_t m, int k_in, int n_out,
                               hipStream_t stream) {
  if (m == 0) return SS_OK;
  if (!ss_wgrad8_ok(m, k_in, n_out, 1)) return SS_ERR_ARG;
  const int nblocks = ss_div_up(m, 64);
  int tm, tn, min_per, splits;
  w8_linear_plan(m, k_in, n_out, &tm, &tn, &min_per, &splits);
  dim3 g((unsigned)(splits * tm * tn));
  SS_LAUNCH((k_wgrad8<false>), g, dim3(512), 0, stream, (const unsigned short*)x, (const unsigned short*)dy,
            (const int32_t*)nullptr, (const int32_t*)nullptr, (const int32_t*)nullptr, (const int32_t*)nullptr, dweight,
            dbias, (int)m, k_in, n_out, 1, tn, nblocks, min_per, tm * tn, splits, 0);
  return SS_OK;
}
```

### scenesplat_amd/functional.py

```python
import os
import weakref

import torch
from torch.utils.weak import WeakIdKeyDictionary

from . import native as nv


class _WindowAttention(torch.autograd.Function):
    @staticmethod
    def forward(ctx, qkv, win, num_heads, scale, impl):
        qkv = qkv.contiguous()
        out, lse = nv.window_attn_fwd(qkv, win, num_heads, scale, impl)
        ctx.save_for_backward(qkv, out, lse)
        ctx.win, ctx.num_heads, ctx.scale, ctx.impl = win, num_heads, scale, impl
        return out

    @staticmethod
    def backward(ctx, dout):
        qkv, out, lse = ctx.saved_tensors
        dqkv = nv.window_attn_bwd(qkv, out, dout.contiguous().to(qkv.dtype), lse, ctx.win, ctx.num_heads, ctx.scale, ctx.impl)
        return dqkv, None, None, None, None


# ... 53 lines not shown


def segment_minmax(src, level, is_max):
    return _SegmentMinMax.apply(src, level, is_max)


def segment_mean(src, level, mean=True):
    return _SegmentMean.apply(src, level, mean)


class _UnpoolAdd(torch.autograd.Function):
    @staticmethod
    def forward(ctx, skip, up, level):
        ctx.level = level
        return nv.gather_add_rows(skip.contiguous(), up.contiguous(), level.cluster)

    @staticmethod
    def backward(ctx, g):
        lv = ctx.level
        g = g.contiguous()
        return g, nv.segment_reduce(g, lv.indices, lv.idx_ptr, lv.n, False), None


def unpool_add(skip, up, level):
    return _UnpoolAdd.apply(skip, up, level)


class _SubMConv3d(torch.autograd.Function):

    @staticmethod
    def forward(ctx, feat, weight, bias, nbr, has_dup, compute_dtype):
        taps, n = nbr.shape
        cout = weight.shape[0]
        x = feat.to(compute_dtype).contiguous()
        w = weight.reshape(cout, taps, -1).to(compute_dtype)
        out = torch.zeros((n, cout), dtype=compute_dtype, device=feat.device) if bias is None else \
            bias.to(compute_dtype).unsqueeze(0).repeat(n, 1)
        buf = torch.empty_like(x)
        for t in range(taps):
            nv.gather_rows(x, nbr[t], out=buf)
            out.addmm_(buf, w[:, t, :].t())
        ctx.save_for_backward(x, weight, nbr)
        ctx.has_bias, ctx.has_dup, ctx.compute_dtype, ctx.in_dtype = bias is not None, has_dup, compute_dtype, feat.dtype
        return out

    @staticmethod
    def backward(ctx, dout):
        x, weight, nbr = ctx.saved_tensors
        taps, n = nbr.shape
        cout = weight.shape[0]
        cd = ctx.compute_dtype
        g = dout.to(cd).contiguous()
        w = weight.reshape(cout, taps, -1).to(cd)
        dx = dw = db = None
        if ctx.needs_input_grad[0]:
            dx = torch.zeros_like(x)
            if not ctx.has_dup:
                buf = torch.empty_like(g)
                for t in range(taps):
                    nv.gather_rows(g, nbr[t], out=buf)
                    dx.addmm_(buf, w[:, taps - 1 - t, :])
            else:
                for t in range(taps):
                    rows = torch.nonzero(nbr[t] >= 0, as_tuple=True)[0]
                    if rows.numel():
                        dx.index_add_(0, nbr[t][rows].long(), g[rows] @ w[:, t, :])
            dx = dx.to(ctx.in_dtype)
        if ctx.needs_input_grad[1]:
            dw = torch.empty((taps, cout, x.shape[1]), dtype=cd, device=x.device)
            buf = torch.empty_like(x)
            gt = g.t()
            for t in range(taps):
                nv.gather_rows(x, nbr[t], out=buf)
                torch.mm(gt, buf, out=dw[t])
            dw = dw.permute(1, 0, 2).reshape(weight.shape).to(weight.dtype)
        if ctx.has_bias and ctx.needs_input_grad[2]:
            db = g.sum(0).to(weight.dtype)
        return dx, dw, db, None, None, None, None


class _SubMConv3dFused(torch.autograd.Function):

    @staticmethod
    def forward(ctx, feat, weight, bias, nbr, rowperm, blocks_fn, has_dup, walk_fn=None, dup_fn=None):
        taps, n = nbr.shape
        cout, cin = weight.shape[0], weight.shape[-1]
        pad = (-cin) % 8
        ctx.dup_fn = dup_fn
        x = feat.to(torch.bfloat16)
        w = bf16_of(weight).reshape(cout, taps, cin)
        if pad:
            x = torch.nn.functional.pad(x, (0, pad)); w = torch.nn.functional.pad(w, (0, pad))
        x, w = x.contiguous(), w.contiguous()
        ctx.meta = (feat.dtype, weight.dtype, weight.shape, cin, bias is not None)
        ctx.blocks_fn, ctx.has_dup = blocks_fn, has_dup
        ctx.wt = mirrored_of(weight) if not pad else None
        ctx.im2col = n <= CONV_IM2COL_MAX_SITES
        out_dtype = torch.bfloat16 if torch.is_autocast_enabled() else torch.float32
        if ctx.im2col:
            cols = nv.subm_im2col(x, nbr)
            out = torch.nn.functional.linear(cols, w.view(cout, -1), bf16_of(bias))
            ctx.save_for_backward(cols, w, nbr, rowperm)
            return out.to(out_dtype)
        walk = None
        if CONV_WALK_RULEBOOK and walk_fn is not None and rowperm is not None and nv.subm_conv_fwd_uses_pipe(n, cin + pad, cout, taps):
            walk = walk_fn()
        ctx.has_walk = walk is not None
        out = nv.subm_conv_fwd(x, w, None if bias is None else bias.float().contiguous(), nbr, rowperm, out_dtype, nbr_walk=walk)
        ctx.save_for_backward(x, w, nbr, rowperm, *(() if walk is None else (walk,)))
        return out

    @staticmethod
    def backward(ctx, dout):
        x, w, nbr, rowperm = ctx.saved_tensors[:4]
        walk = ctx.saved_tensors[4] if getattr(ctx, "has_walk", False) else None
        in_dtype, w_dtype, w_shape, cin, has_bias = ctx.meta
        g = dout.to(torch.bfloat16).contiguous()
        dx = dw = db = None
        runs = gd = None
        if ctx.has_dup and ctx.needs_input_grad[0]:
            runs = ctx.dup_fn() if ctx.dup_fn is not None else nv.dup_runs_from_rulebook(nbr)
            gd = nv.dup_fold_rows(g, runs)
        if ctx.im2col:
            cols = x
            taps = nbr.shape[0]
            if ctx.needs_input_grad[0]:
                wt = ctx.wt if ctx.wt is not None else nv.subm_weight_mirror(w)
                dx = torch.nn.functional.linear(nv.subm_im2col(g if gd is None else gd, nbr), wt.view(wt.shape[0], -1))
                if runs is not None:
                    nv.dup_zero_rows_(dx, runs)
                dx = dx[:, :cin].to(in_dtype)
            if ctx.needs_input_grad[1]:
                dw = _mm_f32(g.t(), cols).view(w.shape)[:, :, :cin].reshape(w_shape).to(w_dtype)
            if has_bias and ctx.needs_input_grad[2]:
                db = g.sum(0, dtype=torch.float32).to(w_dtype)
            return dx, dw, db, None, None, None, None, None, None
        if ctx.needs_input_grad[0]:
            wt = ctx.wt if ctx.wt is not None else nv.subm_weight_mirror(w)
            dx = nv.subm_conv_fwd(g if gd is None else gd, wt, None, nbr, rowperm, nbr_walk=walk)
            if runs is not None:
                nv.dup_zero_rows_(dx, runs)
            dx = dx[:, :cin].to(in_dtype)
        if ctx.needs_input_grad[1]:
            blocks = ctx.blocks_fn() if ctx.blocks_fn is not None else nv.subm_block_lists(nbr, rowperm)
            dw = nv.subm_conv_wgrad(x, g, nbr, rowperm, blocks, nbr_walk=walk)[:, :, :cin].reshape(w_shape).to(w_dtype)
        if has_bias and ctx.needs_input_grad[2]:
            db = g.sum(0, dtype=torch.float32).to(w_dtype)
        return dx, dw, db, None, None, None, None, None, None


def _split_bf16(t):
    t = t.float()
    hi = t.to(torch.bfloat16)
    return hi, (t - hi.float()).to(torch.bfloat16)


class _SubMConv3dSplit(torch.autograd.Function):

    @staticmethod
    def forward(ctx, feat, weight, bias, nbr, rowperm, blocks_fn, has_dup=False, dup_fn=None):
        taps, n = nbr.shape
        cout, cin = weight.shape[0], weight.shape[-1]
        pad = (-cin) % 8
        ctx.has_dup, ctx.dup_fn = has_dup, dup_fn
        x = feat.float()
        w = weight.float().reshape(cout, taps, cin)
        if pad:
            x = torch.nn.functional.pad(x, (0, pad)); w = torch.nn.functional.pad(w, (0, pad))
        xh, xl = _split_bf16(x)
        wh, wl = _split_bf16(w)
        x3 = torch.cat([xh, xl, xh], 1).contiguous()
        w3 = torch.cat([wh, wh, wl], 2).contiguous()
        out = nv.subm_conv_fwd(x3, w3, None if bias is None else bias.float().contiguous(), nbr, rowperm, torch.float32)
        ctx.save_for_backward(xh, xl, wh, wl, nbr, rowperm)
        ctx.meta = (feat.dtype, weight.dtype, weight.shape, cin, bias is not None)
        ctx.blocks_fn = blocks_fn
        return out

    @staticmethod
    def backward(ctx, dout):
        xh, xl, wh, wl, nbr, rowperm = ctx.saved_tensors
        in_dtype, w_dtype, w_shape, cin, has_bias = ctx.meta
        gh, gl = _split_bf16(dout.contiguous())
        dx = dw = db = None
        if ctx.needs_input_grad[0]:
            wt3 = torch.cat([nv.subm_weight_mirror(wh), nv.subm_weight_mirror(wh), nv.subm_weight_mirror(wl)], 2).contiguous()
            runs = None
            fh, fl = gh, gl
            if ctx.has_dup:
                runs = ctx.dup_fn() if ctx.dup_fn is not None else nv.dup_runs_from_rulebook(nbr)
                fh, fl = _split_bf16(nv.dup_fold_rows(dout.float().contiguous(), runs))
            g3 = torch.cat([fh, fl, fh], 1).contiguous()
            dx = nv.subm_conv_fwd(g3, wt3, None, nbr, rowperm, torch.float32)
            if runs is not None:
                nv.dup_zero_rows_(dx, runs)
            dx = dx[:, :cin].to(in_dtype)
        if ctx.needs_input_grad[1]:
            blocks = ctx.blocks_fn() if ctx.blocks_fn is not None else nv.subm_block_lists(nbr, rowperm)
            cp = xh.shape[1]
            d2 = nv.subm_conv_wgrad(torch.cat([xh, xl], 1).contiguous(), gh, nbr, rowperm, blocks)
            d1 = nv.subm_conv_wgrad(xh, gl, nbr, rowperm, blocks)
            dw = (d2[:, :, :cp] + d2[:, :, cp:] + d1)[:, :, :cin].reshape(w_shape).to(w_dtype)
        if has_bias and ctx.needs_input_grad[2]:
            db = dout.sum(0, dtype=torch.float32).to(w_dtype)
        return dx, dw, db, None, None, None, None, None


class _SubMConv3dF32(torch.autograd.Function):

    @staticmethod
    def forward(ctx, feat, weight, bias, nbr, rowperm, blocks_fn, walk_fn, has_dup=False, dup_fn=None):
        taps, n = nbr.shape
        cout, cin = weight.shape[0], weight.shape[-1]
        cp = 16 if cin <= 16 else 32
        ctx.has_dup, ctx.dup_fn, ctx.plain_nbr = has_dup, dup_fn, nbr
        ctx.orig_nbr = nbr if blocks_fn is None else None
        nbr = walk_fn() if walk_fn is not None else nv.subm_walk_rulebook(nbr, rowperm)
        x = feat.float()
        if cp != cin:
            x = torch.nn.functional.pad(x, (0, cp - cin))
        x = x.contiguous()
        w = weight.float().reshape(cout, taps, cin)
        out = nv.subm_f32_fwd(x, nv.subm_f32_weight_layout(w), None if bias is None else bias.float().contiguous(), nbr, rowperm)
        ctx.save_for_backward(x, w, nbr, rowperm)
        ctx.meta = (feat.dtype, weight.dtype, weight.shape, cin, bias is not None)
        ctx.blocks_fn = blocks_fn
        return out

    @staticmethod
    def backward(ctx, dout):
        x, w, nbr, rowperm = ctx.saved_tensors
        in_dtype, w_dtype, w_shape, cin, has_bias = ctx.meta
        g = dout.float().contiguous()
        dx = dw = db = None
        if ctx.needs_input_grad[0]:
            if ctx.has_dup:
                runs = ctx.dup_fn() if ctx.dup_fn is not None else nv.dup_runs_from_rulebook(ctx.plain_nbr)
                dx = nv.subm_f32_fwd(nv.dup_fold_rows(g, runs), nv.subm_f32_weight_layout(w, mirror=True), None, nbr, rowperm,
                                     winners_only=True).to(in_dtype)
            else:
                dx = nv.subm_f32_fwd(g, nv.subm_f32_weight_layout(w, mirror=True), None, nbr, rowperm).to(in_dtype)
        if ctx.needs_input_grad[1]:
            blocks = ctx.blocks_fn() if ctx.blocks_fn is not None else nv.subm_block_lists(ctx.orig_nbr, rowperm)
            dw = nv.subm_f32_wgrad(x, g, nbr, rowperm, blocks, cin).reshape(w_shape).to(w_dtype)
        if has_bias and ctx.needs_input_grad[2]:
            db = g.sum(0, dtype=torch.float32).to(w_dtype)
        return dx, dw, db, None, None, None, None, None, None


CONV_WALK_RULEBOOK = os.environ.get("SS_CONV_WALK", "1") != "0"
CONV_F32_MFMA = os.environ.get("SS_CONV_F32_MFMA", "1") != "0"
CONV_IM2COL_MAX_SITES = int(os.environ.get("SS_CONV_IM2COL_MAX", "8192"))


def _mm_f32(a, b):
    try:
        return torch.mm(a, b, out_dtype=torch.float32)
    except (RuntimeError, NotImplementedError, TypeError):
        return torch.mm(a, b).float()


def subm_conv3d(feat, weight, bias, nbr, has_dup=False, compute_dtype=torch.float32, rowperm=None, blocks_fn=None, walk_fn=None,
                dup_fn=None):
    if compute_dtype == torch.bfloat16 and weight.shape[0] % 8 == 0:
        return _SubMConv3dFused.apply(feat, weight, bias, nbr, rowperm, blocks_fn, has_dup, walk_fn, dup_fn)
    if compute_dtype == "bf16x3":
        if (CONV_F32_MFMA and weight.shape[0] == 32 and weight.shape[-1] <= 32 and feat.is_cuda
                and (weight.shape[-1] == 32 or not feat.requires_grad)):
            return _SubMConv3dF32.apply(feat, weight, bias, nbr, rowperm, blocks_fn, walk_fn, has_dup, dup_fn)
        if weight.shape[0] % 8 == 0 and feat.is_cuda:
            return _SubMConv3dSplit.apply(feat, weight, bias, nbr, rowperm, blocks_fn, has_dup, dup_fn)
        compute_dtype = torch.float32
    return _SubMConv3d.apply(feat, weight, bias, nbr, has_dup, compute_dtype)


class _Gelu(torch.autograd.Function):

    @staticmethod
    def forward(ctx, x):
        x = x.contiguous()
        ctx.save_for_backward(x)
        return nv.gelu(x)

    @staticmethod
    def backward(ctx, dy):
        (x,) = ctx.saved_tensors
        dy = dy.contiguous().to(x.dtype)
        if not _aligned16(dy):
            dy = dy.clone()
        return nv.gelu(x, dy)


GELU_HIP = os.environ.get("SS_GELU_HIP", "1") != "0"


def _aligned16(t):
    return t.data_ptr() % 16 == 0 and t.storage_offset() * t.element_size() % 16 == 0


def gelu(x):
    if GELU_HIP and x.is_cuda and x.dtype in (torch.float32, torch.bfloat16) and _aligned16(x):
        return _Gelu.apply(x)
    return torch.nn.functional.gelu(x)


def lang_head_release():
    _HEAD_CACHE.clear()


class _LangHead(torch.autograd.Function):

    @staticmethod
    def forward(ctx, feat, target, mask, normalize, want_p):
        feat = feat.contiguous()
        if target is not None:
            target = target.contiguous()
            if target.dtype not in (torch.float32, torch.bfloat16):
                target = target.float()
        p, sums, rowstat = nv.lang_head_fwd(feat, target, mask, normalize, want_p=want_p)
        ctx.save_for_backward(feat, target, mask, rowstat)
        ctx.normalize = normalize
        ctx.set_materialize_grads(False)
        return p, sums

    @staticmethod
    def backward(ctx, dp, dsums):
        feat, target, mask, rowstat = ctx.saved_tensors
        if dp is None and (dsums is None or target is None):
            return None, None, None, None, None
        coef = None
        if target is not None:
            coef = (dsums[:2] if dsums is not None else torch.zeros(2, device=feat.device)).float().contiguous()
        dp = dp.contiguous() if dp is not None else None
        return nv.lang_head_bwd(feat, target, mask, ctx.normalize, rowstat, coef, dp), None, None, None, None


_HEAD_CACHE = {}


def lang_head(feat, target=None, mask=None, normalize=True):
    p, sums = _LangHead.apply(feat, target, mask, normalize, True)
    if target is not None:
        _HEAD_CACHE["last"] = (weakref.ref(p), weakref.ref(target), weakref.ref(mask), target._version, mask._version, sums)
    return p, sums


def lang_head_sums(pred, target, mask):
    ent = _HEAD_CACHE.get("last")
    if ent is not None and ent[0]() is pred and ent[1]() is target and ent[2]() is mask and ent[3] == target._version \
            and ent[4] == mask._version:
        return ent[5]
    _, sums = _LangHead.apply(pred, target, mask, False, False)
    _HEAD_CACHE["last"] = (weakref.ref(pred), weakref.ref(target), weakref.ref(mask), target._version, mask._version, sums)
    return sums
# ... 62 lines not shown
            nv.transpose16_group(pairs)
        pairs = [(d.view(d.shape[0], -1, d.shape[-1]), _SHADOW_M[p]) for p, d in zip(todo_s, todo_d) if p in _SHADOW_M]
        if pairs:
            nv.subm_weight_mirror_group(pairs)


def register_mirrored(weights):
    for p in weights:
        ent = _SHADOW.get(p)
        if ent is None or p.dim() != 5 or p.shape[-1] % 8:
            continue
        cout, cin = p.shape[0], p.shape[-1]
        taps = p.numel() // (cout * cin)
        m = _SHADOW_M.get(p)
        if m is None or m.shape != (cin, taps, cout) or m.device != p.device:
            _SHADOW_M[p] = torch.empty((cin, taps, cout), dtype=torch.bfloat16, device=p.device)
            ent[1] = None


def mirrored_of(p):
    if not isinstance(p, torch.nn.Parameter):
        return None
    m = _SHADOW_M.get(p)
    if m is None:
        return None
    ent = _SHADOW.get(p)
    return m if (ent is not None and _shadow_current(ent, p)) else None


def register_transposed(weights):
    for p in weights:
        ent = _SHADOW.get(p)
        if ent is None or p.dim() != 2:
            continue
        t = _SHADOW_T.get(p)
        if t is None or t.shape != (p.shape[1], p.shape[0]) or t.device != p.device:
            _SHADOW_T[p] = torch.empty((p.shape[1], p.shape[0]), dtype=torch.bfloat16, device=p.device)
            ent[1] = None


def unregister_transposed(weights):
    for p in weights:
        if p in _SHADOW_T:
            del _SHADOW_T[p]


def bf16_t_of(p):
    if not isinstance(p, torch.nn.Parameter):
        return None
    t = _SHADOW_T.get(p)
    if t is None:
        return None
    ent = _SHADOW.get(p)
    return t if (ent is not None and _shadow_current(ent, p)) else None


def bf16_of(p):
    if p is None:
        return None
    if p.dtype == torch.bfloat16:
        return p
    ent = _SHADOW.get(p) if isinstance(p, torch.nn.Parameter) else None
    if ent is not None and _shadow_current(ent, p):
        return ent[0]
    return p.to(torch.bfloat16)


WGRAD_GROUP_MAX_ROWS = int(os.environ.get("SS_WGRAD_GROUP_MAX", str(1 << 22)))
_STAGE = {"cur": None, "route": {}}
_UNFLUSHED = set()


WGRAD_GROUP_MAX_BYTES = int(float(os.environ.get("SS_WGRAD_GROUP_MAX_GIB", "8")) * (1 << 30))


class _WgradStage:
    def __init__(self):
        self.queue = []
        self.redq = []
        self.bytes = 0

    def add(self, x, dy, dw, db):
        self.queue.append((x, dy, dw, db))
        self.bytes += x.numel() * x.element_size() + dy.numel() * dy.element_size()
        if self.bytes > WGRAD_GROUP_MAX_BYTES:
            q, self.queue, self.bytes = self.queue, [], 0
            nv.linear_wgrad_group(q)

    def flush(self):
        _UNFLUSHED.discard(self)
        q, self.queue, self.bytes = self.queue, [], 0
        r, self.redq = self.redq, []
        nv.linear_wgrad_group(q)
        nv.group_partial_sums(r)


class _StageParams(torch.autograd.Function):
    @staticmethod
    def forward(ctx, stage, *params):
        ctx.stage = stage
        ctx.set_materialize_grads(False)
        return tuple(p.view_as(p) for p in params)

    @staticmethod
    def backward(ctx, *grads):
        ctx.stage.flush()
        return (None,) + grads


def stage_begin(linears, n_rows):
    _STAGE["cur"], _STAGE["route"] = None, {}
    if not (WGRAD_GROUP_MAX_ROWS and LINEAR_WGRAD_MIN_ROWS <= n_rows <= WGRAD_GROUP_MAX_ROWS and torch.is_grad_enabled()
            and torch.is_autocast_enabled() and torch.get_autocast_dtype("cuda") == torch.bfloat16):
        return
    params = [p for m in linears for p in (m.weight, m.bias) if p is not None and p.requires_grad and p.dtype == torch.float32 and p.is_cuda]
    if not params:
        return
    stage = _WgradStage()
    aliases = _StageParams.apply(stage, *params)
    _STAGE["cur"], _STAGE["route"] = stage, {id(p): a for p, a in zip(params, aliases)}


def stage_end():
    _STAGE["cur"], _STAGE["route"] = None, {}


def reset_state():
    stage_end()
    _UNFLUSHED.clear()
    _HEAD_CACHE.clear()


def _routed(p):
    a = _STAGE["route"].get(id(p)) if (p is not None and _STAGE["route"]) else None
    return (a, _STAGE["cur"]) if a is not None else (p, None)


class _Linear(torch.autograd.Function):

    @staticmethod
    def forward(ctx, x, weight, bias, w16, b16, stage, w16t=None):
        y = torch.nn.functional.linear(x, w16, b16)
        ctx.save_for_backward(x, w16 if w16t is None else w16t)
        ctx.meta = (weight.dtype, bias is not None)
        ctx.dgrad_nt = w16t is not None
        ctx.stage = stage
        return y

    @staticmethod
    def backward(ctx, dy):
        x, w16 = ctx.saved_tensors
        w_dtype, has_bias = ctx.meta
        dx, dw, db = _linear_backward(x, w16, ctx.dgrad_nt, w_dtype, has_bias, ctx.stage, dy.contiguous(), ctx.needs_input_grad[0],
                                      ctx.needs_input_grad[1], ctx.needs_input_grad[2])
        return dx, dw, db, None, None, None, None


class _LinearGelu(torch.autograd.Function):

    @staticmethod
    def forward(ctx, x, weight, bias, w16, b16, stage, w16t=None):
        u = torch.nn.functional.linear(x, w16, b16)
        ctx.save_for_backward(x, w16 if w16t is None else w16t, u)
        ctx.meta = (weight.dtype, bias is not None)
        ctx.dgrad_nt = w16t is not None
        ctx.stage = stage
        return nv.gelu(u)
# ... 515 lines not shown
```

### scenesplat_amd/native.py

```python
import ctypes

import numpy as np
import torch

from . import _lib, grouped
from ._lib import check

F32, BF16 = 0, 1
ATTN_SIMT, ATTN_MFMA = 0, 1
HAVE_MFMA_ATTN = True
ORDER_IDS = {"z": 0, "z-trans": 1, "hilbert": 2, "hilbert-trans": 3}


def _p(t):
    return ctypes.c_void_p(t.data_ptr()) if t is not None else ctypes.c_void_p(0)


def _stream():
    return ctypes.c_void_p(torch.cuda.current_stream().cuda_stream)


def _req(t, dtype=None, name="tensor", shape=None):
    if not isinstance(t, torch.Tensor) or not t.is_cuda:
        raise RuntimeError(f"{name}: scenesplat_amd ops need a GPU tensor (no CPU fallback)")
# ... 162 lines not shown
    if rowperm is not None:
        _req(rowperm, torch.int32, "rowperm", (n,))
    splits = lib().ss_subm_conv_splits(n, cout, taps)
    if splits > 1:
        acc = torch.zeros((n, cout), dtype=torch.float32, device=x.device)
        check(lib().ss_subm_conv_fwd_splitk(_p(x), _p(w), _p(bias), _p(nbr), _p(rowperm), _p(acc), n, cin, cout, taps, splits,
                                            _stream()), "ss_subm_conv_fwd_splitk")
        return acc if out_dtype == torch.float32 else acc.to(out_dtype)
    out = torch.empty((n, cout), dtype=out_dtype, device=x.device)
    if nbr_walk is not None:
        _req(nbr_walk, torch.int32, "nbr_walk", (taps, n))
        check(lib().ss_subm_conv_fwd_walk(_p(x), _p(w), _p(bias), _p(nbr), _p(nbr_walk), _p(rowperm), _p(out), n, cin, cout, taps,
                                          dtype_code(out), _stream()), "ss_subm_conv_fwd_walk")
        return out
    check(lib().ss_subm_conv_fwd(_p(x), _p(w), _p(bias), _p(nbr), _p(rowperm), _p(out), n, cin, cout, taps,
                                 dtype_code(out), _stream()), "ss_subm_conv_fwd")
    return out


def subm_weight_mirror(w):
    cout, taps, cin = w.shape
    _req(w, torch.bfloat16, "w")
    wt = torch.empty((cin, taps, cout), dtype=torch.bfloat16, device=w.device)
    check(lib().ss_subm_weight_mirror(_p(w), _p(wt), cout, taps, cin, _stream()), "ss_subm_weight_mirror")
    return wt


def subm_im2col(x, nbr):
    n, c = x.shape
    taps = nbr.shape[0]
    _req(x, torch.bfloat16, "x"); _req(nbr, torch.int32, "nbr", (taps, n))
    if c % 8:
        raise RuntimeError("subm_im2col: channels must be a multiple of 8")
    out = torch.empty((n, taps * c), dtype=torch.bfloat16, device=x.device)
    check(lib().ss_subm_im2col(_p(x), _p(nbr), _p(out), n, taps, c * 2, _stream()), "ss_subm_im2col")
    return out


def subm_conv_fwd_pipe(x, w, bias, nbr, rowperm, out_dtype=torch.bfloat16):
    n, cin = x.shape
    cout, taps = w.shape[0], w.shape[1]
    out = torch.empty((n, cout), dtype=out_dtype, device=x.device)
    check(lib().ss_subm_conv_fwd_pipe(_p(x), _p(w), _p(bias), _p(nbr), _p(rowperm), _p(out), n, cin, cout, taps,
                                      dtype_code(out), _stream()), "ss_subm_conv_fwd_pipe")
    return out


def linear_fwd(x, w, bias=None, out_dtype=torch.bfloat16):
    m, k = x.shape
    n = w.shape[0]
    out = torch.empty((m, n), dtype=out_dtype, device=x.device)
    check(lib().ss_linear_fwd(_p(x), _p(w), _p(bias), _p(out), m, k, n, dtype_code(out), _stream()), "ss_linear_fwd")
    return out


def subm_block_lists(nbr, rowperm):
    taps, n = nbr.shape
    _req(nbr, torch.int32, "nbr")
    if rowperm is not None:
        _req(rowperm, torch.int32, "rowperm", (n,))
    nb = (n + 63) // 64
    cnt = torch.empty(taps, dtype=torch.int32, device=nbr.device)
    lst = torch.empty((taps, nb), dtype=torch.int32, device=nbr.device)
    check(lib().ss_subm_block_lists(_p(nbr), _p(rowperm), n, taps, _p(cnt), _p(lst), _stream()), "ss_subm_block_lists")
    return cnt, lst


_ARENA = {"buf": None, "off": 0}


def zero_arena_begin(numel, device):
    _ARENA["buf"] = torch.zeros(int(numel), dtype=torch.float32, device=device) if numel > 0 else None
    _ARENA["off"] = 0


def zeros_f32(numel, device):
    buf, off = _ARENA["buf"], _ARENA["off"]
    if buf is not None and buf.device == device and off + numel <= buf.numel():
        _ARENA["off"] = off + ((numel + 3) & ~3)
        return buf[off:off + numel]
    return torch.zeros(int(numel), dtype=torch.float32, device=device)


def subm_conv_wgrad(x, dout, nbr, rowperm, blocks, out=None, nbr_walk=None):
    n, cin = x.shape
    cout = dout.shape[1]
    taps = nbr.shape[0]
    _req(x, torch.bfloat16, "x"); _req(dout, torch.bfloat16, "dout", (n, cout)); _req(nbr, torch.int32, "nbr", (taps, n))
    if cin % 8 or cout % 8:
        raise RuntimeError("subm_conv_wgrad: channels must be multiples of 8")
    if rowperm is not None:
        _req(rowperm, torch.int32, "rowperm", (n,))
    dw = zeros_f32(cout * taps * cin, x.device).view(cout, taps, cin) if out is None else _req(out, torch.float32, "out", (cout, taps, cin))
    cnt, lst = blocks
    _req(cnt, torch.int32, "blk_count", (taps,)); _req(lst, torch.int32, "blk_list", (taps, (n + 63) // 64))
    if nbr_walk is not None:
        _req(nbr_walk, torch.int32, "nbr_walk", (taps, n))
    check(lib().ss_subm_conv_wgrad_walk(_p(x), _p(dout), _p(nbr), _p(nbr_walk), _p(rowperm), _p(cnt), _p(lst), _p(dw), n, cin, cout, taps,
                                        _stream()), "ss_subm_conv_wgrad")
    return dw


def subm_f32_weight_layout(w, mirror=False):
    w = w.float()
    if mirror:
        w = w.flip(1).permute(2, 1, 0)
    co, taps, c = w.shape
    cp = 16 if c <= 16 else 32
    if co != 32 or c > 32:
        raise RuntimeError("subm_f32: 32 output channels, at most 32 input channels")
    if cp != c:
        w = torch.nn.functional.pad(w, (0, cp - c))
    return w.reshape(32, taps, cp // 8, 2, 4).permute(1, 2, 3, 0, 4).contiguous()


def subm_walk_rulebook(nbr, rowperm):
    return nbr if rowperm is None else nbr.index_select(1, rowperm).contiguous()


def subm_f32_fwd(x, wq, bias, nbr, rowperm, winners_only=False):
    n, cp = x.shape
    taps = nbr.shape[0]
    _req(x, torch.float32, "x"); _req(wq, torch.float32, "wq", (taps, cp // 8, 2, 32, 4)); _req(nbr, torch.int32, "nbr", (taps, n))
    if bias is not None:
        _req(bias, torch.float32, "bias", (32,))
    if rowperm is not None:
        _req(rowperm, torch.int32, "rowperm", (n,))
    out = torch.empty((n, 32), dtype=torch.float32, device=x.device)
    if winners_only:
        if bias is not None:
            raise RuntimeError("subm_f32_fwd: the dgrad form takes no bias")
        check(lib().ss_subm_f32_dgrad_dup(_p(x), _p(wq), _p(nbr), _p(rowperm), _p(out), n, cp, 32, taps, _stream()), "ss_subm_f32_dgrad_dup")
        return out
    check(lib().ss_subm_f32_fwd(_p(x), _p(wq), _p(bias), _p(nbr), _p(rowperm), _p(out), n, cp, 32, taps, _stream()), "ss_subm_f32_fwd")
    return out


def dup_runs_from_rulebook(nbr):
    keys, order = torch.sort(nbr[nbr.shape[0] // 2].long(), stable=True)
    return keys.contiguous(), order.to(torch.int32).contiguous()


def dup_fold_rows(src, runs):
    keys, order = runs
    n, C = src.shape
    _req(src, None, "src"); _req(keys, torch.int64, "sorted_keys", (n,)); _req(order, torch.int32, "order", (n,))
    out = torch.empty_like(src)
    check(lib().ss_dup_fold_rows(_p(src), _p(keys), _p(order), _p(out), n, C, dtype_code(src), _stream()), "ss_dup_fold_rows")
    return out


def dup_zero_rows_(x, runs):
    keys, order = runs
    n = x.shape[0]
    _req(x, None, "x"); _req(keys, torch.int64, "sorted_keys", (n,)); _req(order, torch.int32, "order", (n,))
    check(lib().ss_dup_zero_rows(_p(keys), _p(order), _p(x), n, x.shape[1] * x.element_size(), _stream()), "ss_dup_zero_rows")
    return x


def subm_f32_wgrad(x, dout, nbr, rowperm, blocks, cin):
    n, cp = x.shape
    taps = nbr.shape[0]
    _req(x, torch.float32, "x"); _req(dout, torch.float32, "dout", (n, 32)); _req(nbr, torch.int32, "nbr", (taps, n))
    if rowperm is not None:
        _req(rowperm, torch.int32, "rowperm", (n,))
    cnt, lst = blocks
    _req(cnt, torch.int32, "blk_count", (taps,)); _req(lst, torch.int32, "blk_list", (taps, (n + 63) // 64))
    dw = zeros_f32(32 * taps * cin, x.device).view(32, taps, cin)
    check(lib().ss_subm_f32_wgrad(_p(x), _p(dout), _p(nbr), _p(rowperm), _p(cnt), _p(lst), _p(dw), n, cp, cin, 32, taps, _stream()),
          "ss_subm_f32_wgrad")
    return dw


def subm_conv_wgrad_pipe(x, dout, nbr, rowperm, blocks):
    n, cin = x.shape
    cout, taps = dout.shape[1], nbr.shape[0]
    dw = torch.zeros((cout, taps, cin), dtype=torch.float32, device=x.device)
    cnt, lst = blocks
    check(lib().ss_subm_conv_wgrad_pipe(_p(x), _p(dout), _p(nbr), _p(rowperm), _p(cnt), _p(lst), _p(dw), n, cin, cout, taps,
                                        _stream()), "ss_subm_conv_wgrad_pipe")
    return dw


def linear_wgrad_alloc(k, nout, want_bias, device):
    buf = zeros_f32(nout * k + (nout if want_bias else 0), device)
    return buf[:nout * k].view(nout, k), (buf[nout * k:] if want_bias else None)


def linear_wgrad_into(x, dy, dw, db):
    m, k = x.shape
    nout = dy.shape[1]
    _req(x, torch.bfloat16, "x"); _req(dy, torch.bfloat16, "dy", (m, nout)); _req(dw, torch.float32, "dw", (nout, k))
    check(lib().ss_linear_wgrad(_p(x), _p(dy), _p(dw), _p(db), m, k, nout, _stream()), "ss_linear_wgrad")


def linear_wgrad_group(items):
    if not items:
        return
    dev = items[0][0].device
    desc = np.zeros((len(items), 8), dtype=np.int64)
    counts = []
    launch_tiles = sum(lib().ss_linear_wgrad_tiles(x.shape[1], dy.shape[1]) for x, dy, _, _ in items)
    for x, dy, dw, db in items:
        _req(x, torch.bfloat16, "x"); _req(dy, torch.bfloat16, "dy", (x.shape[0], dy.shape[1]))
        _req(dw, torch.float32, "dw", (dy.shape[1], x.shape[1]))
        if db is not None:
            _req(db, torch.float32, "db", (dy.shape[1],))
        j = len(counts)
        nwg = lib().ss_linear_wgrad_group_plan2(x.shape[0], x.shape[1], dy.shape[1], launch_tiles, ctypes.c_void_p(desc[j].ctypes.data))
        if nwg <= 0 or j >= 128:
            linear_wgrad_into(x, dy, dw, db)
            continue
        desc[j, 0], desc[j, 1], desc[j, 2] = x.data_ptr(), dy.data_ptr(), dw.data_ptr()
        desc[j, 3] = db.data_ptr() if db is not None else 0
        desc[j, 4] = x.shape[0]
        counts.append(nwg)
    if counts:
        grouped.launch("ss_linear_wgrad_group", desc[:len(counts)].copy(), grouped.starts(counts), dev)


def linear_wgrad(x, dy, want_bias=False):
    m, k = x.shape
    nout = dy.shape[1]
    _req(x, torch.bfloat16, "x"); _req(dy, torch.bfloat16, "dy", (m, nout))
    buf = zeros_f32(nout * k + (nout if want_bias else 0), x.device)
    dw = buf[:nout * k].view(nout, k)
    db = buf[nout * k:] if want_bias else None
    check(lib().ss_linear_wgrad(_p(x), _p(dy), _p(dw), _p(db), m, k, nout, _stream()), "ss_linear_wgrad")
    return (dw, db) if want_bias else dw


def _dt(t):
    return dtype_code(t) if t is not None else 0


def add_layernorm_fwd(x, y, rowscale, gamma, beta, eps, want_xout, want_copy, h_dtype):
    n, C = x.shape
    _req(x, None, "x")
    if y is not None:
        _req(y, None, "y", (n, C))
    if rowscale is not None:
        _req(rowscale, torch.float32, "rowscale", (n,))
    dev = x.device
    xout = torch.empty((n, C), dtype=torch.float32, device=dev) if want_xout else None
    xcopy = torch.empty((n, C), dtype=torch.bfloat16, device=dev) if want_copy else None
    h = mean = rstd = None
    if gamma is not None:
        _req(gamma, torch.float32, "gamma", (C,)); _req(beta, torch.float32, "beta", (C,))
        h = torch.empty((n, C), dtype=h_dtype, device=dev)
        mean = torch.empty(n, dtype=torch.float32, device=dev); rstd = torch.empty(n, dtype=torch.float32, device=dev)
    check(lib().ss_add_layernorm_fwd(_p(x), _dt(x), _p(y), _dt(y), _p(rowscale), _p(gamma), _p(beta), float(eps), _p(xout), F32,
                                     _p(xcopy), _p(h), _dt(h), _p(mean), _p(rstd), n, C, _stream()), "ss_add_layernorm_fwd")
    return xout, xcopy, h, mean, rstd


def ln_add_ln_fwd(x, t, gamma0, beta0, eps0, gamma1, beta1, eps1, h_dtype):
    n, C = x.shape
    _req(x, None, "x"); _req(t, None, "t", (n, C))
    for p_, nm in ((gamma0, "gamma0"), (beta0, "beta0"), (gamma1, "gamma1"), (beta1, "beta1")):
        _req(p_, torch.float32, nm, (C,))
    dev = x.device
    xout = torch.empty((n, C), dtype=torch.float32, device=dev)
    h = torch.empty((n, C), dtype=h_dtype, device=dev)
    stats = torch.empty((n, 4), dtype=torch.float32, device=dev)
    check(lib().ss_ln_add_ln_fwd(_p(x), _dt(x), _p(t), _dt(t), _p(gamma0), _p(beta0), float(eps0), _p(gamma1), _p(beta1), float(eps1),
                                 _p(xout), _p(h), _dt(h), _p(stats), n, C, _stream()), "ss_ln_add_ln_fwd")
    return xout, h, stats


def group_partial_sums(items):
    if not items:
        return
    dev = items[0][0].device
    desc = np.zeros((len(items), 4), dtype=np.int64)
    per = lib().ss_group_partial_sums_outputs_per_workgroup()
    for j, (part, dst) in enumerate(items):
        K, nb, C = part.shape
        _req(part, torch.float32, "part"); _req(dst, torch.float32, "dst", (K, C))
        desc[j] = (part.data_ptr(), dst.data_ptr(), nb, C | ((K * C) << 32))
    grouped.launch("ss_group_partial_sums", desc, grouped.starts(_div_up(desc[:, 3] >> 32, per)), dev)


def subm_weight_mirror_group(pairs):
    if not pairs:
        return
    dev = pairs[0][0].device
# ... 917 lines not shown
```

### scenesplat_amd/pointcept_api/ptv3.py

```python
import os
from functools import partial

import torch
import torch.nn as nn
import torch.nn.functional as F

from .. import functional as SF
from .. import native as nv
from ..plan import build_plan
from .pdnorm import PDNorm, PointModule, ResolvedNorm, pdnorm_layers, resolved as _rn
from .registry import MODELS
from .structure import Point

RUNTIME = dict(attn_impl=nv.ATTN_SIMT, conv_dtype=None,
               attn_headmajor=os.environ.get("SS_ATTN_HM", "1") != "0",
               param_shadows=os.environ.get("SS_PARAM_SHADOWS", "1") != "0",
               fuse_block_tail=os.environ.get("SS_BLOCK_TAIL", "1") != "0")


def bench_runtime():
    return dict(attn_impl=nv.ATTN_MFMA, conv_dtype=torch.bfloat16,
                conv_split_max_channels=int(os.environ.get("SS_CONV_SPLIT_MAX", "32")))


def conv_wants_walk(n_sites, channels, ksize):
    cin, cout = channels if isinstance(channels, (tuple, list)) else (channels, channels)
    cd = conv_dtype_for(cout)
    if cd == "bf16x3":
        return bool(SF.CONV_F32_MFMA and cout == 32 and cin <= 32)
    if cd == torch.bfloat16 and cout % 8 == 0:
        return bool(SF.CONV_WALK_RULEBOOK and n_sites > SF.CONV_IM2COL_MAX_SITES
                    and nv.subm_conv_fwd_uses_pipe(n_sites, cin + (-cin) % 8, cout, ksize ** 3))
    return False


def conv_dtype_for(out_channels):
    cd = RUNTIME["conv_dtype"] or torch.float32
    if cd == torch.bfloat16 and out_channels <= RUNTIME.get("conv_split_max_channels", 0):
        return "bf16x3"
    return cd


class DropPath(nn.Module):

    def __init__(self, p=0.0):
        super().__init__()
        self.p = float(p)

    def forward(self, x):
        if self.p == 0.0 or not self.training:
            return x
        keep = 1.0 - self.p
        mask = x.new_empty((x.shape[0], 1)).bernoulli_(keep)
        if keep > 0.0:
            mask.div_(keep)
        return x * mask


class SubMConv3d(nn.Module):

    def __init__(self, in_channels, out_channels, kernel_size, bias=True, indice_key=None):
        super().__init__()
        k = kernel_size
        self.kernel_size, self.indice_key = k, indice_key
        self.weight = nn.Parameter(torch.empty(out_channels, k, k, k, in_channels))
        self.bias = nn.Parameter(torch.zeros(out_channels)) if bias else None
        nn.init.kaiming_uniform_(self.weight.view(out_channels, -1), a=5 ** 0.5)

    def forward(self, feat, level):
        cd = conv_dtype_for(self.weight.shape[0])
        return SF.subm_conv3d(feat, self.weight, self.bias, level.neighbors(self.kernel_size),
                              level.has_duplicates, cd, level.conv_rowperm(),
                              lambda: level.conv_blocks(self.kernel_size), lambda: level.neighbors_walk(self.kernel_size),
                              level.dup_runs)


def _lin(mod, x):
    return SF.linear(x, mod.weight, mod.bias)


class RPE(nn.Module):

    def __init__(self, patch_size, num_heads):
        super().__init__()
        self.patch_size, self.num_heads = patch_size, num_heads
        self.pos_bnd = int((4 * patch_size) ** (1 / 3) * 2)
        self.rpe_num = 2 * self.pos_bnd + 1
        self.rpe_table = nn.Parameter(torch.zeros(3 * self.rpe_num, num_heads))
        nn.init.trunc_normal_(self.rpe_table, std=0.02)


class SerializedAttention(PointModule):
    def __init__(self, channels, num_heads, patch_size, qkv_bias=True, qk_scale=None, attn_drop=0.0,
                 proj_drop=0.0, order_index=0, enable_rpe=False, enable_flash=True, upcast_attention=True,
                 upcast_softmax=True):
        super().__init__()
        assert channels % num_heads == 0
        if enable_rpe and enable_flash:
            raise AssertionError("Set enable_rpe to False when enable Flash Attention")
        if attn_drop != 0.0 or proj_drop != 0.0:
            raise NotImplementedError("attention / projection dropout are 0 in the reference configs")
        self.channels, self.num_heads, self.patch_size = channels, num_heads, patch_size
        self.scale = qk_scale or (channels // num_heads) ** -0.5
        self.order_index = order_index
        self.enable_rpe = bool(enable_rpe)
        self.qkv = nn.Linear(channels, channels * 3, bias=qkv_bias)
        self.proj = nn.Linear(channels, channels)
        self.rpe = RPE(patch_size, num_heads) if enable_rpe else None

    def rpe_window_size(self, level):
        k = min(min(level.counts), self.patch_size)
        if k < 1:
            raise ValueError("enable_rpe: every batch element needs at least one point")
        return k

    def _forward_rpe(self, x, level, pre_proj=False):
        win = level.window(self.order_index, self.rpe_window_size(level))
        qkv = _lin(self.qkv, x)
        bf16 = (x.is_cuda and torch.is_autocast_enabled() and torch.get_autocast_dtype("cuda") == torch.bfloat16) \
            or qkv.dtype == torch.bfloat16
        if bf16 and (self.channels // self.num_heads) in (16, 32, 48, 64):
            impl = nv.ATTN_MFMA
        else:
            impl = nv.ATTN_SIMT
        a = qkv.to(torch.bfloat16) if bf16 else qkv
        feat = SF.window_attention_rpe(a, win, level.grid_coord, self.rpe.rpe_table, self.rpe.pos_bnd, self.num_heads,
                                       self.scale, impl).to(qkv.dtype)
        return feat if pre_proj else _lin(self.proj, feat)

    def forward(self, x, level, pre_proj=False):
        if self.enable_rpe:
            return self._forward_rpe(x, level, pre_proj)
        win = level.window(self.order_index, self.patch_size)
        impl = RUNTIME["attn_impl"]
        if (impl == nv.ATTN_MFMA and RUNTIME.get("attn_headmajor", True) and x.is_cuda and torch.is_autocast_enabled()
                and torch.get_autocast_dtype("cuda") == torch.bfloat16 and self.qkv.weight.dtype == torch.float32
                and (self.channels // self.num_heads) in (16, 32, 48, 64)):
            feat = SF.qkv_window_attention(x, self.qkv.weight, self.qkv.bias, win, self.num_heads, self.scale)
            return feat if pre_proj else _lin(self.proj, feat)
        qkv = _lin(self.qkv, x)
        if impl == nv.ATTN_MFMA and qkv.dtype != torch.bfloat16:
            feat = SF.window_attention(qkv.to(torch.bfloat16), win, self.num_heads, self.scale, impl).to(qkv.dtype)
        else:
            feat = SF.window_attention(qkv, win, self.num_heads, self.scale, impl)
        return feat if pre_proj else _lin(self.proj, feat)


class MLP(nn.Module):
    def __init__(self, in_channels, hidden_channels=None, out_channels=None, act_layer=nn.GELU, drop=0.0):
        super().__init__()
        out_channels = out_channels or in_channels
        hidden_channels = hidden_channels or in_channels
        self.fc1 = nn.Linear(in_channels, hidden_channels)
        self.act = act_layer()
        self.fc2 = nn.Linear(hidden_channels, out_channels)

    def forward(self, x):
# ... 206 lines not shown
        blk = dict(mlp_ratio=mlp_ratio, qkv_bias=qkv_bias, qk_scale=qk_scale, attn_drop=attn_drop, proj_drop=proj_drop,
                   norm_layer=ln_layer, act_layer=act_layer, pre_norm=pre_norm, enable_rpe=enable_rpe,
                   enable_flash=enable_flash, upcast_attention=upcast_attention, upcast_softmax=upcast_softmax)
        enc_dp = [x.item() for x in torch.linspace(0, drop_path, sum(enc_depths))]
        self.enc = _Stage()
        for s in range(self.num_stages):
            dp = enc_dp[sum(enc_depths[:s]):sum(enc_depths[:s + 1])]
            enc = _Stage()
            if s > 0:
                enc.down = SerializedPooling(enc_channels[s - 1], enc_channels[s], stride[s - 1], bn_layer, act_layer)
            for i in range(enc_depths[s]):
                setattr(enc, f"block{i}", Block(enc_channels[s], enc_num_head[s], enc_patch_size[s], drop_path=dp[i],
                                               order_index=i % len(self.order), cpe_indice_key=f"stage{s}", **blk))
            setattr(self.enc, f"enc{s}", enc)
        self.enc_depths, self.dec_depths = tuple(enc_depths), tuple(dec_depths)
        if not cls_mode:
            dec_dp = [x.item() for x in torch.linspace(0, drop_path, sum(dec_depths))]
            self.dec = _Stage()
            dec_channels = list(dec_channels) + [enc_channels[-1]]
            for s in reversed(range(self.num_stages - 1)):
                dp = dec_dp[sum(dec_depths[:s]):sum(dec_depths[:s + 1])]
                dp.reverse()
                dec = _Stage()
                dec.up = SerializedUnpooling(dec_channels[s + 1], enc_channels[s], dec_channels[s], bn_layer, act_layer)
                for i in range(dec_depths[s]):
                    setattr(dec, f"block{i}", Block(dec_channels[s], dec_num_head[s], dec_patch_size[s], drop_path=dp[i],
                                                   order_index=i % len(self.order), cpe_indice_key=f"stage{s}", **blk))
                setattr(self.dec, f"dec{s}", dec)

    def draw_perms(self):
        K = len(self.order)
        perms = [torch.randperm(K).tolist() if self.shuffle_orders else list(range(K))]
        for s in range(1, self.num_stages):
            down = getattr(self.enc, f"enc{s}").down
            perms.append(torch.randperm(K).tolist() if down.shuffle_orders else list(range(K)))
        return perms

    def plan_specs(self, with_dec=True):
        K = len(self.order)
        with_dec = with_dec and not self.cls_mode
        wide = list(self.enc_channels)
        if with_dec:
            for s, c in enumerate(self.dec_channels_):
                wide[s] = max(wide[s], c)
        walk = [[c for c in {self.enc_channels[s], wide[s]}] for s in range(self.num_stages)]
        wins, ks = [], [(0, 5, [(self.embedding.in_channels, self.enc_channels[0])])]
        for s in range(self.num_stages):
            enc = getattr(self.enc, f"enc{s}")
            ks.append((s, 3, walk[s]))
            for i in range(self.enc_depths[s]):
                attn = getattr(enc, f"block{i}").attn
                if not attn.enable_rpe:
                    wins.append((s, i % K, attn.patch_size))
        if with_dec:
            for s in range(self.num_stages - 1):
                dec = getattr(self.dec, f"dec{s}")
                for i in range(self.dec_depths[s]):
                    attn = getattr(dec, f"block{i}").attn
                    if not attn.enable_rpe:
                        wins.append((s, i % K, attn.patch_size))
        return wins, ks

    def prepare_plan(self, data_dict, perms=None, stream=None, with_dec=True):
        if "grid_coord" not in data_dict:
            raise KeyError("prepare_plan needs grid_coord")
        perms = perms if perms is not None else self.draw_perms()
        if stream is None:
            plan = build_plan(data_dict["grid_coord"], data_dict["offset"], self.order, self.stride, perms)
            plan.materialize(*self.plan_specs(with_dec))
            return plan
        with torch.cuda.stream(stream):
            plan = build_plan(data_dict["grid_coord"], data_dict["offset"], self.order, self.stride, perms)
            plan.materialize(*self.plan_specs(with_dec))
            plan.ready_event = torch.cuda.Event()
            plan.ready_event.record(stream)
        return plan

    def _stage_linears(self, stage):
        cache = self.__dict__.setdefault("_stage_linear_cache", {})
        ls = cache.get(id(stage))
        if ls is None:
            skip = self._modulation_linears()
            ls = [m for m in stage.modules() if isinstance(m, (nn.Linear, nn.LayerNorm)) and id(m) not in skip]
            cache[id(stage)] = ls
        return ls

    def _refresh_shadows(self):
        ps = self.__dict__.get("_shadow_lists")
        tail = SF.BLOCK_TAIL_MAX_CHANNELS if RUNTIME.get("fuse_block_tail", True) else 0
        if ps is None or ps[2] != next(self.parameters()).device or ps[4] != tail:
            params, skip = [], self._modulation_linears()
            for m in self.modules():
                if isinstance(m, nn.Linear) and id(m) not in skip:
                    params += [m.weight, m.bias]
                elif isinstance(m, SubMConv3d):
                    params += [m.weight, m.bias]
            src, dst = SF.register_shadows(params)
            wide = []
            for st in [getattr(self.enc, f"enc{s}", None) for s in (0, 1)] + [getattr(getattr(self, "dec", None), f"dec{s}", None) for s in (0, 1)]:
                if st is not None:
                    wide += [m.weight for m in st.modules() if isinstance(m, nn.Linear) and m.weight.numel() >= 65536]
            if RUNTIME.get("dgrad_nt", True):
                SF.register_transposed(wide)
            keep = {id(w) for w in wide} if RUNTIME.get("dgrad_nt", True) else set()
            mine = [w for m in self.modules() if isinstance(m, Block) and m.channels in SF.BLOCK_TAIL_CHANNELS and m.channels <= tail
                    and m.pre_norm and not isinstance(m.norm2[0], PDNorm)
                    and tuple(m.mlp[0].fc1.weight.shape) == (4 * m.channels, m.channels)
                    for w in (m.attn.proj.weight, m.mlp[0].fc1.weight, m.mlp[0].fc2.weight) if id(w) not in keep]
            SF.unregister_transposed([w for w in self.__dict__.get("_tail_transposed", []) if id(w) not in {id(v) for v in mine}])
            SF.register_transposed(mine)
            self.__dict__["_tail_transposed"] = mine
            SF.register_mirrored([m.weight for m in self.modules() if isinstance(m, SubMConv3d)
                                  and conv_dtype_for(m.weight.shape[0]) == torch.bfloat16])
            total = sum(((p.numel() + 3) & ~3) for p in params if p is not None) + 4 * len(params)
            ps = (src, dst, next(self.parameters()).device, total, tail)
            self.__dict__["_shadow_lists"] = ps
        SF.refresh_shadows(ps[0], ps[1])
        if torch.is_grad_enabled():
            nv.zero_arena_begin(ps[3], ps[2])

    def _pdnorm(self):
        pds = self.__dict__.get("_pdnorm_list")
        if pds is None:
            pds = self.__dict__["_pdnorm_list"] = pdnorm_layers(self)
        return pds

    def _modulation_linears(self):
        return {id(m.modulation[1]) for m in self._pdnorm() if m.adaptive}

    def _resolve_pdnorm(self, point):
        pds = self._pdnorm()
        assert "condition" in point.keys(), f"feat and condition must be in point.keys(): {point.keys()}"
        idx = pds[0].index_of(point["condition"])
        if not pds[0].adaptive:
            for m in pds:
                m.__dict__["_resolved"] = m.resolve_static(idx)
            return
        assert "context" in point.keys()
        split = (not self.cls_mode and torch.is_grad_enabled() and point.get("backward_cut", None) is not None)
        cache = self.__dict__.setdefault("_pdnorm_groups", {})
        groups = cache.get((idx, split))
        if groups is None:
            last = {id(m) for m in pdnorm_layers(self.dec.dec0)} if not self.cls_mode else set()
            parts = [[m for m in pds if id(m) not in last], [m for m in pds if id(m) in last]]
            if not split:
                parts = [(parts[0] + parts[1], len(parts[0]))]
            else:
                parts = [(ms, 0) for ms in parts if ms]
            groups = cache[(idx, split)] = [(ms, SF.PDNormGroup([m.row(idx) for m in ms], sp)) for ms, sp in parts]
        for ms, group in groups:
            for m, (g, b) in zip(ms, SF.pdnorm_modulation(group, point["context"])):
                m.__dict__["_resolved"] = ResolvedNorm(g, b, m.norm[idx])

    def _draw_row_scales(self, levels, device, with_dec=True):
        blocks = []
        for s in range(self.num_stages):
            enc = getattr(self.enc, f"enc{s}")
            blocks += [(getattr(enc, f"block{i}"), levels[s].n) for i in range(self.enc_depths[s])]
        if not self.cls_mode and with_dec:
            for s in reversed(range(self.num_stages - 1)):
                dec = getattr(self.dec, f"dec{s}")
                blocks += [(getattr(dec, f"block{i}"), levels[s].n) for i in range(self.dec_depths[s])]
        segs = []
        for blk, n in blocks:
            dp = blk.drop_path[0]
            if isinstance(dp, DropPath) and dp.p > 0.0:
# ... 108 lines not shown
```

Before: 2.881 million.

## Fuse sparse-conv bias gradient into weight-gradient kernels via ones-MFMA at center tap

Adds bias-gradient accumulation to the submanifold conv weight-gradient kernels (bf16 MFMA, pipelined, and f32 paths). At the center tap every output row is visited exactly once, so summing dout there gives dbias. Bias-only problems can also be added to the grouped linear wgrad launch. This removes separate torch reductions over dout for conv biases, at the cost of extra MFMAs and atomics in one tap's workgroups and a bias-only path in the grouped kernel. It is enabled by default through an environment flag.

```diff
diff --git a/include/scenesplat_hip.h b/include/scenesplat_hip.h
--- a/include/scenesplat_hip.h
+++ b/include/scenesplat_hip.h
@@ -158,6 +158,16 @@
 int ss_subm_conv_wgrad_walk(const void* in, const void* dout, const int32_t* nbr, const int32_t* nbr_walk, const int32_t* rowperm,
                             const int32_t* blk_count, const int32_t* blk_list, float* dweight, int64_t n, int cin, int cout,
                             int taps, ss_stream_t stream);
+int ss_subm_conv_wgrad_bias(const void* in, const void* dout, const int32_t* nbr, const int32_t* nbr_walk, const int32_t* rowperm,
+                            const int32_t* blk_count, const int32_t* blk_list, float* dweight, float* dbias, int64_t n, int cin,
+                            int cout, int taps, ss_stream_t stream);
+int ss_subm_conv_wgrad_pipe_bias(const void* in, const void* dout, const int32_t* nbr, const int32_t* rowperm,
+                                 const int32_t* blk_count, const int32_t* blk_list, float* dweight, float* dbias, int64_t n,
+                                 int cin, int cout, int taps, int walk, ss_stream_t stream);
+int ss_subm_f32_wgrad_bias(const float* in, const float* dout, const int32_t* nbr_walk, const int32_t* rowperm,
+                           const int32_t* blk_count, const int32_t* blk_list, float* dweight, float* dbias, int64_t n,
+                           int cin_padded, int cin, int cout, int taps, ss_stream_t stream);
+int ss_linear_wgrad_group_plan_bias(int64_t m, int n_out, int64_t* desc_words);
 
 int ss_add_layernorm_fwd(const void* x, int x_dtype, const void* y, int y_dtype, const float* rowscale,
                          const float* gamma, const float* beta, float eps, void* xout, int xout_dtype, void* xcopy_bf16,
diff --git a/scenesplat_amd/_lib.py b/scenesplat_amd/_lib.py
--- a/scenesplat_amd/_lib.py
+++ b/scenesplat_amd/_lib.py
@@ -86,6 +86,10 @@
     "ss_subm_conv_wgrad_pipe_walk": (c_i, [c_p, c_p, c_p, c_p, c_p, c_p, c_p, c_i64, c_i, c_i, c_i, c_p]),
     "ss_subm_conv_wgrad_uses_pipe": (c_i, [c_i64, c_i, c_i, c_i]),
     "ss_subm_conv_wgrad_walk": (c_i, [c_p, c_p, c_p, c_p, c_p, c_p, c_p, c_p, c_i64, c_i, c_i, c_i, c_p]),
+    "ss_subm_conv_wgrad_bias": (c_i, [c_p, c_p, c_p, c_p, c_p, c_p, c_p, c_p, c_p, c_i64, c_i, c_i, c_i, c_p]),
+    "ss_subm_conv_wgrad_pipe_bias": (c_i, [c_p, c_p, c_p, c_p, c_p, c_p, c_p, c_p, c_i64, c_i, c_i, c_i, c_i, c_p]),
+    "ss_subm_f32_wgrad_bias": (c_i, [c_p, c_p, c_p, c_p, c_p, c_p, c_p, c_p, c_i64, c_i, c_i, c_i, c_i, c_p]),
+    "ss_linear_wgrad_group_plan_bias": (c_i, [c_i64, c_i, c_p]),
     "ss_subm_f32_ok": (c_i, [c_i, c_i]),
     "ss_subm_f32_fwd": (c_i, [c_p, c_p, c_p, c_p, c_p, c_p, c_i64, c_i, c_i, c_i, c_p]),
     "ss_subm_f32_dgrad_dup": (c_i, [c_p, c_p, c_p, c_p, c_p, c_i64, c_i, c_i, c_i, c_p]),
diff --git a/scenesplat_amd/csrc/subm_conv.hip b/scenesplat_amd/csrc/subm_conv.hip
--- a/scenesplat_amd/csrc/subm_conv.hip
+++ b/scenesplat_amd/csrc/subm_conv.hip
@@ -251,12 +251,12 @@
   return SS_OK;
 }
 
-template <int WM, int WN, int TM, int TN>
+template <int WM, int WN, int TM, int TN, bool BIAS>
 __global__ void __launch_bounds__(64 * WM * WN)
 k_subm_wgrad(const unsigned short* __restrict__ in, const unsigned short* __restrict__ dout,
              const int32_t* __restrict__ nbr, const int32_t* __restrict__ rowperm, const int32_t* __restrict__ blk_count,
-             const int32_t* __restrict__ blk_list, float* __restrict__ dW, int n, int Cin, int Cout, int taps, int ntiles_n,
-             int nblocks_total) {
+             const int32_t* __restrict__ blk_list, float* __restrict__ dW, float* __restrict__ dbias, int n, int Cin, int Cout,
+             int taps, int ntiles_n, int nblocks_total) {
   constexpr int THREADS = 64 * WM * WN, BMc = 16 * TM * WM, BNc = 16 * TN * WN;
   constexpr int ARB = BMc * 2, BRB = BNc * 2;
   constexpr int AIMG = 64 * ARB, BIMG = 64 * BRB;
@@ -280,6 +280,17 @@
   for (int mi = 0; mi < TM; ++mi)
 #pragma unroll
     for (int ni = 0; ni < TN; ++ni) acc[mi][ni] = f32x4_t{0.f, 0.f, 0.f, 0.f};
+  constexpr int BM = TM / WN;
+  const bool do_bias = BIAS && n0 == 0 && tap == taps / 2;
+  const int wnu = __builtin_amdgcn_readfirstlane(wn);
+  f32x4_t accb[BM];
+#pragma unroll
+  for (int q = 0; q < BM; ++q) accb[q] = f32x4_t{0.f, 0.f, 0.f, 0.f};
+  bf8_t ones;
+  {
+    s8_t o = {0x3F80, 0x3F80, 0x3F80, 0x3F80, 0x3F80, 0x3F80, 0x3F80, 0x3F80};
+    ones = __builtin_bit_cast(bf8_t, o);
+  }
   uint4 sa[NLA], sb[NLB];
   auto index_load = [&](int b, int blk) {
     if (tid < 64) {
@@ -344,6 +355,16 @@
         for (int mi = 0; mi < TM; ++mi)
 #pragma unroll
           for (int ni = 0; ni < TN; ++ni) acc[mi][ni] = MFMA16(af[mi], bf[ni], acc[mi][ni]);
+        if (do_bias) {
+#pragma unroll
+          for (int q = 0; q < BM; ++q) {
+            bf8_t a = af[q];
+#pragma unroll
+            for (int w = 1; w < WN; ++w)
+              if (wnu == w) a = af[w * BM + q];
+            accb[q] = MFMA16(a, ones, accb[q]);
+          }
+        }
       }
     }
     __syncthreads();
@@ -364,6 +385,15 @@
         }
       }
     }
+  if (do_bias && lq == 0) {
+#pragma unroll
+    for (int q = 0; q < BM; ++q)
+#pragma unroll
+      for (int r = 0; r < 4; ++r) {
+        int co = m0 + 16 * TM * wm + 16 * (wnu * BM + q) + 4 * g + r;
+        if (co < Cout) atomicAdd(dbias + co, accb[q][r]);
+      }
+  }
 }
 
 template <typename OutT>
@@ -445,25 +475,31 @@
 }
 extern "C" int ss_subm_conv_wgrad_uses_pipe(int64_t n, int cin, int cout, int taps) { return conv_wgrad_uses_pipe(n, cin, cout, taps) ? 1 : 0; }
 
-extern "C" int ss_subm_conv_wgrad_walk(const void* in, const void* dout, const int32_t* nbr, const int32_t* nbr_walk,
+extern "C" int ss_subm_conv_wgrad_bias(const void* in, const void* dout, const int32_t* nbr, const int32_t* nbr_walk,
                                        const int32_t* rowperm, const int32_t* blk_count, const int32_t* blk_list, float* dweight,
-                                       int64_t n, int cin, int cout, int taps, hipStream_t stream);
+                                       float* dbias, int64_t n, int cin, int cout, int taps, hipStream_t stream);
 
 extern "C" int ss_subm_conv_wgrad(const void* in, const void* dout, const int32_t* nbr, const int32_t* rowperm,
                                   const int32_t* blk_count, const int32_t* blk_list, float* dweight, int64_t n, int cin,
                                   int cout, int taps, hipStream_t stream) {
-  return ss_subm_conv_wgrad_walk(in, dout, nbr, nullptr, rowperm, blk_count, blk_list, dweight, n, cin, cout, taps, stream);
+  return ss_subm_conv_wgrad_bias(in, dout, nbr, nullptr, rowperm, blk_count, blk_list, dweight, nullptr, n, cin, cout, taps, stream);
 }
 
 extern "C" int ss_subm_conv_wgrad_walk(const void* in, const void* dout, const int32_t* nbr, const int32_t* nbr_walk,
                                        const int32_t* rowperm, const int32_t* blk_count, const int32_t* blk_list, float* dweight,
                                        int64_t n, int cin, int cout, int taps, hipStream_t stream) {
+  return ss_subm_conv_wgrad_bias(in, dout, nbr, nbr_walk, rowperm, blk_count, blk_list, dweight, nullptr, n, cin, cout, taps, stream);
+}
+
+extern "C" int ss_subm_conv_wgrad_bias(const void* in, const void* dout, const int32_t* nbr, const int32_t* nbr_walk,
+                                       const int32_t* rowperm, const int32_t* blk_count, const int32_t* blk_list, float* dweight,
+                                       float* dbias, int64_t n, int cin, int cout, int taps, hipStream_t stream) {
   if (n < 0 || cin <= 0 || cout <= 0 || taps <= 0 || (cin & 7) || (cout & 7) || n >= (1LL << 31)) return SS_ERR_ARG;
+  if (dbias && !(taps & 1)) return SS_ERR_ARG;
   if (n == 0) return SS_OK;
-  if (conv_wgrad_uses_pipe(n, cin, cout, taps)) {
-    if (nbr_walk) return ss_subm_conv_wgrad_pipe_walk(in, dout, nbr_walk, rowperm, blk_count, blk_list, dweight, n, cin, cout, taps, stream);
-    return ss_subm_conv_wgrad_pipe(in, dout, nbr, rowperm, blk_count, blk_list, dweight, n, cin, cout, taps, stream);
-  }
+  if (conv_wgrad_uses_pipe(n, cin, cout, taps))
+    return ss_subm_conv_wgrad_pipe_bias(in, dout, nbr_walk ? nbr_walk : nbr, rowperm, blk_count, blk_list, dweight, dbias, n, cin, cout,
+                                        taps, nbr_walk ? 1 : 0, stream);
   const int nblocks = ss_div_up(n, 64);
   const bool big = cout >= 256 && cin >= 256 && nblocks >= 1024;
   const int T = big ? 256 : 128;
@@ -473,9 +509,9 @@
   if (splits < 1) splits = 1;
   dim3 g(tm * tn, taps, splits);
   const unsigned short* x = (const unsigned short*)in; const unsigned short* go = (const unsigned short*)dout;
-  if (big)
-    SS_LAUNCH((k_subm_wgrad<2, 4, 8, 4>), g, dim3(512), 0, stream, x, go, nbr, rowperm, blk_count, blk_list, dweight, (int)n, cin, cout, taps, tn, nblocks);
-  else
-    SS_LAUNCH((k_subm_wgrad<2, 2, 4, 4>), g, dim3(256), 0, stream, x, go, nbr, rowperm, blk_count, blk_list, dweight, (int)n, cin, cout, taps, tn, nblocks);
+#define CV_WGRAD(WN, TM, THREADS, BIAS) SS_LAUNCH((k_subm_wgrad<2, WN, TM, 4, BIAS>), g, dim3(THREADS), 0, stream, x, go, nbr, rowperm, blk_count, blk_list, dweight, dbias, (int)n, cin, cout, taps, tn, nblocks)
+  if (big) { if (dbias) CV_WGRAD(4, 8, 512, true); else CV_WGRAD(4, 8, 512, false); }
+  else { if (dbias) CV_WGRAD(2, 4, 256, true); else CV_WGRAD(2, 4, 256, false); }
+#undef CV_WGRAD
   return SS_OK;
 }
diff --git a/scenesplat_amd/csrc/subm_f32.hip b/scenesplat_amd/csrc/subm_f32.hip
--- a/scenesplat_amd/csrc/subm_f32.hip
+++ b/scenesplat_amd/csrc/subm_f32.hip
@@ -98,11 +98,11 @@
 
 #define SF_WPER 4
 
-template <int CI>
+template <int CI, bool BIAS>
 __global__ void __launch_bounds__(256) __attribute__((amdgpu_waves_per_eu(3, 3)))
 k_subm_f32_wgrad(const float* __restrict__ in, const float* __restrict__ g, const int32_t* __restrict__ nbr_walk,
                  const int32_t* __restrict__ rowperm, const int32_t* __restrict__ blk_count, const int32_t* __restrict__ blk_list,
-                 float* __restrict__ dW, int n, int taps, int cin, int nblocks) {
+                 float* __restrict__ dW, float* __restrict__ dbias, int n, int taps, int cin, int nblocks) {
   constexpr int NCH = CI / 4;
   constexpr int NX = (32 * NCH) / 64;
   constexpr int WAVE_LDS = 2 * SF_WPER * 64 * 4 + 32 * 128 + 32 * CI * 4;
@@ -146,6 +146,8 @@
   f32x16_t acc;
 #pragma unroll
   for (int r = 0; r < 16; ++r) acc[r] = 0.f;
+  const bool do_bias = BIAS && tap == taps / 2;
+  float bsum = 0.f;
   auto consume = [&](const float4 (&rg)[4], const float4 (&rx)[NX]) {
 #pragma unroll
     for (int r = 0; r < 4; ++r) {
@@ -162,6 +164,7 @@
       const float a = *reinterpret_cast<const float*>(gimg + (2 * u + kk) * 128 + j * 4);
       const float x = *reinterpret_cast<const float*>(ximg + (2 * u + kk) * (CI * 4) + (j & (CI - 1)) * 4);
       acc = F32MFMA(a, x, acc);
+      if (do_bias) bsum += a;
     }
   };
   {
@@ -182,6 +185,10 @@
       atomicAdd(dW + ((int64_t)co * taps + tap) * cin + j, acc[r]);
     }
   }
+  if (do_bias) {
+    bsum += __shfl_xor(bsum, 32, 64);
+    if (kk == 0) atomicAdd(dbias + j, bsum);
+  }
 }
 
 extern "C" int ss_subm_f32_ok(int cin_padded, int cout) { return cout == 32 && (cin_padded == 16 || cin_padded == 32); }
@@ -207,16 +214,25 @@
   return subm_f32_launch(dout_folded, wq, nullptr, nbr_walk, rowperm, din, n, cin_padded, cout, taps, taps / 2, stream);
 }
 
+extern "C" int ss_subm_f32_wgrad_bias(const float* in, const float* gout, const int32_t* nbr_walk, const int32_t* rowperm,
+                                      const int32_t* blk_count, const int32_t* blk_list, float* dweight, float* dbias, int64_t n,
+                                      int cin_padded, int cin, int cout, int taps, hipStream_t stream);
 extern "C" int ss_subm_f32_wgrad(const float* in, const float* gout, const int32_t* nbr_walk, const int32_t* rowperm,
                                  const int32_t* blk_count, const int32_t* blk_list, float* dweight, int64_t n, int cin_padded,
                                  int cin, int cout, int taps, hipStream_t stream) {
+  return ss_subm_f32_wgrad_bias(in, gout, nbr_walk, rowperm, blk_count, blk_list, dweight, nullptr, n, cin_padded, cin, cout, taps, stream);
+}
+extern "C" int ss_subm_f32_wgrad_bias(const float* in, const float* gout, const int32_t* nbr_walk, const int32_t* rowperm,
+                                      const int32_t* blk_count, const int32_t* blk_list, float* dweight, float* dbias, int64_t n,
+                                      int cin_padded, int cin, int cout, int taps, hipStream_t stream) {
+  if (dbias && !(taps & 1)) return SS_ERR_ARG;
   if (n < 0 || n >= (1LL << 31) || taps <= 0 || !ss_subm_f32_ok(cin_padded, cout) || cin <= 0 || cin > cin_padded) return SS_ERR_ARG;
   if (n == 0) return SS_OK;
   const int nblocks = ss_div_up(n, 64);
   dim3 g(ss_div_up(ss_div_up(nblocks, SF_WPER), 4), taps), b(256);
-  if (cin_padded == 16)
-    SS_LAUNCH((k_subm_f32_wgrad<16>), g, b, 0, stream, in, gout, nbr_walk, rowperm, blk_count, blk_list, dweight, (int)n, taps, cin, nblocks);
-  else
-    SS_LAUNCH((k_subm_f32_wgrad<32>), g, b, 0, stream, in, gout, nbr_walk, rowperm, blk_count, blk_list, dweight, (int)n, taps, cin, nblocks);
+#define SF_WGRAD(CI, BIAS) SS_LAUNCH((k_subm_f32_wgrad<CI, BIAS>), g, b, 0, stream, in, gout, nbr_walk, rowperm, blk_count, blk_list, dweight, dbias, (int)n, taps, cin, nblocks)
+  if (cin_padded == 16) { if (dbias) SF_WGRAD(16, true); else SF_WGRAD(16, false); }
+  else { if (dbias) SF_WGRAD(32, true); else SF_WGRAD(32, false); }
+#undef SF_WGRAD
   return SS_OK;
 }
diff --git a/scenesplat_amd/csrc/wgrad8.hip b/scenesplat_amd/csrc/wgrad8.hip
--- a/scenesplat_amd/csrc/wgrad8.hip
+++ b/scenesplat_amd/csrc/wgrad8.hip
@@ -59,7 +59,9 @@
 #pragma unroll
         for (int ni = 0; ni < 2; ++ni) acc[a][mi][b][ni] = f32x4_t{0.f, 0.f, 0.f, 0.f};
 
-  const bool do_bias = !GATHER && dbias != nullptr && (tile % ntn) == 0;
+  const bool bias_wg = dbias != nullptr && (!GATHER || tap == taps / 2);
+  const bool do_bias0 = bias_wg && (tile % ntn) == 0;
+  const bool do_bias1 = bias_wg && (tile % ntn) == ((GATHER && ntn > 1) ? 1 : 0);
   f32x4_t accb[2] = {f32x4_t{0.f, 0.f, 0.f, 0.f}, f32x4_t{0.f, 0.f, 0.f, 0.f}};
   w8_bf8_t ones;
   {
@@ -150,7 +152,7 @@
   _Pragma("unroll") for (int ni = 0; ni < 2; ++ni)                                                \
       acc[HA][mi][HB][ni] = W8_MFMA(af[mi][ks], BF[ni][ks], acc[HA][mi][HB][ni]);
 #define W8_BIAS(HA)                                                                               \
-  if (do_bias) {                                                                                  \
+  if (HA ? do_bias1 : do_bias0) {                                                                            \
     if (wc == 0) { accb[HA] = W8_MFMA(af[0][0], ones, accb[HA]); accb[HA] = W8_MFMA(af[0][1], ones, accb[HA]); }       \
     else if (wc == 1) { accb[HA] = W8_MFMA(af[1][0], ones, accb[HA]); accb[HA] = W8_MFMA(af[1][1], ones, accb[HA]); }  \
     else if (wc == 2) { accb[HA] = W8_MFMA(af[2][0], ones, accb[HA]); accb[HA] = W8_MFMA(af[2][1], ones, accb[HA]); }  \
@@ -264,13 +266,15 @@
             if (ci < Cin) atomicAdd(rowp + ci, acc[ha][mi][hb][ni][r]);
           }
       }
-  if (do_bias && lq == 0) {
+  if (lq == 0) {
 #pragma unroll
     for (int ha = 0; ha < 2; ++ha)
-#pragma unroll
-      for (int r = 0; r < 4; ++r) {
-        const int co = m0 + 128 * wr + 64 * ha + 16 * wc + 4 * g + r;
-        if (co < Cout) atomicAdd(dbias + co, accb[ha][r]);
+      if (ha ? do_bias1 : do_bias0) {
+#pragma unroll
+        for (int r = 0; r < 4; ++r) {
+          const int co = m0 + 128 * wr + 64 * ha + 16 * wc + 4 * g + r;
+          if (co < Cout) atomicAdd(dbias + co, accb[ha][r]);
+        }
       }
   }
 }
@@ -297,6 +301,29 @@
                   nshares, L, walk & 1);
 }
 
+__device__ __forceinline__ void w8_bias_only(const unsigned short* __restrict__ dy, float* __restrict__ dbias, int m, int n_out,
+                                             int per, int L) {
+  const int nch = n_out >> 3;
+  const int rl = 512 / nch, tid = threadIdx.x;
+  if (tid >= rl * nch) return;
+  const int c = tid % nch, r0 = tid / nch;
+  const int64_t beg = (int64_t)L * per * 64, end = min((int64_t)m, beg + (int64_t)per * 64);
+  float s[8] = {0.f, 0.f, 0.f, 0.f, 0.f, 0.f, 0.f, 0.f};
+  for (int64_t r = beg + r0; r < end; r += rl) {
+    const uint4 v = *reinterpret_cast<const uint4*>(dy + r * n_out + c * 8);
+    const unsigned w[4] = {v.x, v.y, v.z, v.w};
+#pragma unroll
+    for (int q = 0; q < 4; ++q) {
+      s[2 * q] += __uint_as_float(w[q] << 16);
+      s[2 * q + 1] += __uint_as_float(w[q] & 0xffff0000u);
+    }
+  }
+  if (beg + r0 < end) {
+#pragma unroll
+    for (int q = 0; q < 8; ++q) atomicAdd(dbias + c * 8 + q, s[q]);
+  }
+}
+
 __global__ void __launch_bounds__(512)
 k_wgrad8_group(const int64_t* __restrict__ desc, const int32_t* __restrict__ wg_start, int nprob, int nprob_flags) {
   const int b = blockIdx.x;
@@ -307,6 +334,10 @@
   const int k_in = (int)(w5 & 0xffffffffu), n_out = (int)(w5 >> 32);
   const int ntn = (int)(w6 & 0xffffffffu), ntiles = (int)(w6 >> 32);
   const int nshares = (int)(w7 & 0xffffffffu), min_per = (int)(w7 >> 32);
+  if (d[0] == 0) {
+    w8_bias_only((const unsigned short*)d[1], (float*)d[3], (int)m, n_out, min_per, b - wg_start[p]);
+    return;
+  }
   int L = b - wg_start[p];
   if (nprob_flags & 1) {
     const int a = (8 - (wg_start[p] & 7)) & 7;
@@ -336,21 +367,29 @@
 }
 
 static int w8_conv_launch(const void* in, const void* dout, const int32_t* nbr, const int32_t* rowperm, const int32_t* blk_count,
-                          const int32_t* blk_list, float* dweight, int64_t n, int cin, int cout, int taps, int walk, hipStream_t stream);
+                          const int32_t* blk_list, float* dweight, float* dbias, int64_t n, int cin, int cout, int taps, int walk,
+                          hipStream_t stream);
 
 extern "C" int ss_subm_conv_wgrad_pipe(const void* in, const void* dout, const int32_t* nbr, const int32_t* rowperm,
                                        const int32_t* blk_count, const int32_t* blk_list, float* dweight, int64_t n,
                                        int cin, int cout, int taps, hipStream_t stream) {
-  return w8_conv_launch(in, dout, nbr, rowperm, blk_count, blk_list, dweight, n, cin, cout, taps, 0, stream);
+  return w8_conv_launch(in, dout, nbr, rowperm, blk_count, blk_list, dweight, nullptr, n, cin, cout, taps, 0, stream);
 }
 extern "C" int ss_subm_conv_wgrad_pipe_walk(const void* in, const void* dout, const int32_t* nbr_walk, const int32_t* rowperm,
                                             const int32_t* blk_count, const int32_t* blk_list, float* dweight, int64_t n,
                                             int cin, int cout, int taps, hipStream_t stream) {
-  return w8_conv_launch(in, dout, nbr_walk, rowperm, blk_count, blk_list, dweight, n, cin, cout, taps, 1, stream);
+  return w8_conv_launch(in, dout, nbr_walk, rowperm, blk_count, blk_list, dweight, nullptr, n, cin, cout, taps, 1, stream);
+}
+extern "C" int ss_subm_conv_wgrad_pipe_bias(const void* in, const void* dout, const int32_t* nbr, const int32_t* rowperm,
+                                            const int32_t* blk_count, const int32_t* blk_list, float* dweight, float* dbias,
+                                            int64_t n, int cin, int cout, int taps, int walk, hipStream_t stream) {
+  if (dbias && !(taps & 1)) return SS_ERR_ARG;
+  return w8_conv_launch(in, dout, nbr, rowperm, blk_count, blk_list, dweight, dbias, n, cin, cout, taps, walk ? 1 : 0, stream);
 }
 
 static int w8_conv_launch(const void* in, const void* dout, const int32_t* nbr, const int32_t* rowperm, const int32_t* blk_count,
-                          const int32_t* blk_list, float* dweight, int64_t n, int cin, int cout, int taps, int walk, hipStream_t stream) {
+                          const int32_t* blk_list, float* dweight, float* dbias, int64_t n, int cin, int cout, int taps, int walk,
+                          hipStream_t stream) {
   if (n == 0) return SS_OK;
   if (!ss_wgrad8_ok(n, cin, cout, taps) || !blk_count || !blk_list || !nbr) return SS_ERR_ARG;
   const int nblocks = ss_div_up(n, 64);
@@ -362,7 +401,7 @@
   if (ss_wgrad_xcd_order()) walk |= 2;
   dim3 g((unsigned)((int64_t)taps * splits * tm * tn));
   SS_LAUNCH((k_wgrad8<true>), g, dim3(512), 0, stream, (const unsigned short*)in, (const unsigned short*)dout, nbr, rowperm,
-            blk_count, blk_list, dweight, (float*)nullptr, (int)n, cin, cout, taps, tn, nblocks, min_per, tm * tn, splits, walk);
+            blk_count, blk_list, dweight, dbias, (int)n, cin, cout, taps, tn, nblocks, min_per, tm * tn, splits, walk);
   return SS_OK;
 }
 
@@ -398,6 +437,15 @@
   return ss_linear_wgrad_group_plan2(m, k_in, n_out, 0, desc_words);
 }
 
+extern "C" int ss_linear_wgrad_group_plan_bias(int64_t m, int n_out, int64_t* desc_words) {
+  if (m <= 0 || m >= (1LL << 31) || n_out < 8 || (n_out & 7) || n_out > W8_ZERO_ELEMS || !desc_words) return 0;
+  const int nblocks = ss_div_up(m, 64), per = 8, splits = ss_div_up(nblocks, per);
+  desc_words[5] = (int64_t)((uint64_t)(uint32_t)n_out << 32);
+  desc_words[6] = (int64_t)((uint64_t)1u << 32);
+  desc_words[7] = (int64_t)((uint64_t)(uint32_t)splits | ((uint64_t)(uint32_t)per << 32));
+  return splits;
+}
+
 extern "C" int ss_linear_wgrad_group(const int64_t* desc, const int32_t* wg_start, int nprob, int total_workgroups,
                                      hipStream_t stream) {
   SS_GROUP_GUARD(desc, wg_start, nprob, total_workgroups);
diff --git a/scenesplat_amd/functional.py b/scenesplat_amd/functional.py
--- a/scenesplat_amd/functional.py
+++ b/scenesplat_amd/functional.py
@@ -159,11 +159,13 @@
 class _SubMConv3dFused(torch.autograd.Function):
 
     @staticmethod
-    def forward(ctx, feat, weight, bias, nbr, rowperm, blocks_fn, has_dup, walk_fn=None, dup_fn=None):
+    def forward(ctx, feat, weight, bias, nbr, rowperm, blocks_fn, has_dup, walk_fn=None, dup_fn=None, b16=None, stage=None,
+                dbias_hip=False):
         taps, n = nbr.shape
         cout, cin = weight.shape[0], weight.shape[-1]
         pad = (-cin) % 8
         ctx.dup_fn = dup_fn
+        ctx.stage, ctx.dbias_hip = stage, bool(dbias_hip) and taps % 2 == 1
         x = feat.to(torch.bfloat16)
         w = bf16_of(weight).reshape(cout, taps, cin)
         if pad:
@@ -176,7 +178,7 @@
         out_dtype = torch.bfloat16 if torch.is_autocast_enabled() else torch.float32
         if ctx.im2col:
             cols = nv.subm_im2col(x, nbr)
-            out = torch.nn.functional.linear(cols, w.view(cout, -1), bf16_of(bias))
+            out = torch.nn.functional.linear(cols, w.view(cout, -1), b16 if b16 is not None else bf16_of(bias))
             ctx.save_for_backward(cols, w, nbr, rowperm)
             return out.to(out_dtype)
         walk = None
@@ -210,8 +212,16 @@
             if ctx.needs_input_grad[1]:
                 dw = _mm_f32(g.t(), cols).view(w.shape)[:, :, :cin].reshape(w_shape).to(w_dtype)
             if has_bias and ctx.needs_input_grad[2]:
-                db = g.sum(0, dtype=torch.float32).to(w_dtype)
-            return dx, dw, db, None, None, None, None, None, None
+                if ctx.dbias_hip and w_dtype == torch.float32 and g.data_ptr() % 16 == 0:
+                    db = nv.zeros_f32(g.shape[1], g.device)
+                    if ctx.stage is not None:
+                        ctx.stage.add(None, g, None, db)
+                    else:
+                        nv.bias_wgrad_into(g, db)
+                else:
+                    db = g.sum(0, dtype=torch.float32).to(w_dtype)
+            return (dx, dw, db) + (None,) * 9
+        want_db = has_bias and ctx.needs_input_grad[2]
         if ctx.needs_input_grad[0]:
             wt = ctx.wt if ctx.wt is not None else nv.subm_weight_mirror(w)
             dx = nv.subm_conv_fwd(g if gd is None else gd, wt, None, nbr, rowperm, nbr_walk=walk)
@@ -220,10 +230,15 @@
             dx = dx[:, :cin].to(in_dtype)
         if ctx.needs_input_grad[1]:
             blocks = ctx.blocks_fn() if ctx.blocks_fn is not None else nv.subm_block_lists(nbr, rowperm)
-            dw = nv.subm_conv_wgrad(x, g, nbr, rowperm, blocks, nbr_walk=walk)[:, :, :cin].reshape(w_shape).to(w_dtype)
-        if has_bias and ctx.needs_input_grad[2]:
+            if want_db and ctx.dbias_hip:
+                dw, db = nv.subm_conv_wgrad(x, g, nbr, rowperm, blocks, nbr_walk=walk, dbias=True)
+                db, want_db = db.to(w_dtype), False
+            else:
+                dw = nv.subm_conv_wgrad(x, g, nbr, rowperm, blocks, nbr_walk=walk)
+            dw = dw[:, :, :cin].reshape(w_shape).to(w_dtype)
+        if want_db:
             db = g.sum(0, dtype=torch.float32).to(w_dtype)
-        return dx, dw, db, None, None, None, None, None, None
+        return (dx, dw, db) + (None,) * 9
 
 
 def _split_bf16(t):
@@ -235,11 +250,12 @@
 class _SubMConv3dSplit(torch.autograd.Function):
 
     @staticmethod
-    def forward(ctx, feat, weight, bias, nbr, rowperm, blocks_fn, has_dup=False, dup_fn=None):
+    def forward(ctx, feat, weight, bias, nbr, rowperm, blocks_fn, has_dup=False, dup_fn=None, dbias_hip=False):
         taps, n = nbr.shape
         cout, cin = weight.shape[0], weight.shape[-1]
         pad = (-cin) % 8
         ctx.has_dup, ctx.dup_fn = has_dup, dup_fn
+        ctx.dbias_hip = bool(dbias_hip) and taps % 2 == 1
         x = feat.float()
         w = weight.float().reshape(cout, taps, cin)
         if pad:
@@ -275,22 +291,28 @@
         if ctx.needs_input_grad[1]:
             blocks = ctx.blocks_fn() if ctx.blocks_fn is not None else nv.subm_block_lists(nbr, rowperm)
             cp = xh.shape[1]
-            d2 = nv.subm_conv_wgrad(torch.cat([xh, xl], 1).contiguous(), gh, nbr, rowperm, blocks)
-            d1 = nv.subm_conv_wgrad(xh, gl, nbr, rowperm, blocks)
+            if has_bias and ctx.needs_input_grad[2] and ctx.dbias_hip:
+                d2, db = nv.subm_conv_wgrad(torch.cat([xh, xl], 1).contiguous(), gh, nbr, rowperm, blocks, dbias=True)
+                d1, db = nv.subm_conv_wgrad(xh, gl, nbr, rowperm, blocks, dbias=db)
+                db = db.to(w_dtype)
+            else:
+                d2 = nv.subm_conv_wgrad(torch.cat([xh, xl], 1).contiguous(), gh, nbr, rowperm, blocks)
+                d1 = nv.subm_conv_wgrad(xh, gl, nbr, rowperm, blocks)
             dw = (d2[:, :, :cp] + d2[:, :, cp:] + d1)[:, :, :cin].reshape(w_shape).to(w_dtype)
-        if has_bias and ctx.needs_input_grad[2]:
+        if has_bias and ctx.needs_input_grad[2] and db is None:
             db = dout.sum(0, dtype=torch.float32).to(w_dtype)
-        return dx, dw, db, None, None, None, None, None
+        return dx, dw, db, None, None, None, None, None, None
 
 
 class _SubMConv3dF32(torch.autograd.Function):
 
     @staticmethod
-    def forward(ctx, feat, weight, bias, nbr, rowperm, blocks_fn, walk_fn, has_dup=False, dup_fn=None):
+    def forward(ctx, feat, weight, bias, nbr, rowperm, blocks_fn, walk_fn, has_dup=False, dup_fn=None, dbias_hip=False):
         taps, n = nbr.shape
         cout, cin = weight.shape[0], weight.shape[-1]
         cp = 16 if cin <= 16 else 32
         ctx.has_dup, ctx.dup_fn, ctx.plain_nbr = has_dup, dup_fn, nbr
+        ctx.dbias_hip = bool(dbias_hip) and taps % 2 == 1
         ctx.orig_nbr = nbr if blocks_fn is None else None
         nbr = walk_fn() if walk_fn is not None else nv.subm_walk_rulebook(nbr, rowperm)
         x = feat.float()
@@ -319,15 +341,21 @@
                 dx = nv.subm_f32_fwd(g, nv.subm_f32_weight_layout(w, mirror=True), None, nbr, rowperm).to(in_dtype)
         if ctx.needs_input_grad[1]:
             blocks = ctx.blocks_fn() if ctx.blocks_fn is not None else nv.subm_block_lists(ctx.orig_nbr, rowperm)
-            dw = nv.subm_f32_wgrad(x, g, nbr, rowperm, blocks, cin).reshape(w_shape).to(w_dtype)
-        if has_bias and ctx.needs_input_grad[2]:
+            if has_bias and ctx.needs_input_grad[2] and ctx.dbias_hip:
+                dw, db = nv.subm_f32_wgrad(x, g, nbr, rowperm, blocks, cin, want_bias=True)
+                db = db.to(w_dtype)
+            else:
+                dw = nv.subm_f32_wgrad(x, g, nbr, rowperm, blocks, cin)
+            dw = dw.reshape(w_shape).to(w_dtype)
+        if has_bias and ctx.needs_input_grad[2] and db is None:
             db = g.sum(0, dtype=torch.float32).to(w_dtype)
-        return dx, dw, db, None, None, None, None, None, None
+        return dx, dw, db, None, None, None, None, None, None, None
 
 
 CONV_WALK_RULEBOOK = os.environ.get("SS_CONV_WALK", "1") != "0"
 CONV_F32_MFMA = os.environ.get("SS_CONV_F32_MFMA", "1") != "0"
 CONV_IM2COL_MAX_SITES = int(os.environ.get("SS_CONV_IM2COL_MAX", "8192"))
+CONV_DBIAS_HIP = os.environ.get("SS_CONV_DBIAS_HIP", "1") != "0"
 
 
 def _mm_f32(a, b):
@@ -338,15 +366,22 @@
 
 
 def subm_conv3d(feat, weight, bias, nbr, has_dup=False, compute_dtype=torch.float32, rowperm=None, blocks_fn=None, walk_fn=None,
-                dup_fn=None):
+                dup_fn=None, dbias_hip=None):
+    dbh = (CONV_DBIAS_HIP if dbias_hip is None else bool(dbias_hip)) and feat.is_cuda
     if compute_dtype == torch.bfloat16 and weight.shape[0] % 8 == 0:
-        return _SubMConv3dFused.apply(feat, weight, bias, nbr, rowperm, blocks_fn, has_dup, walk_fn, dup_fn)
+        b16 = stage = None
+        br = bias
+        if dbh and bias is not None and nbr.shape[1] <= CONV_IM2COL_MAX_SITES and torch.is_grad_enabled():
+            br, stage = _routed(bias)
+            if stage is not None:
+                b16 = bf16_of(bias)
+        return _SubMConv3dFused.apply(feat, weight, br, nbr, rowperm, blocks_fn, has_dup, walk_fn, dup_fn, b16, stage, dbh)
     if compute_dtype == "bf16x3":
         if (CONV_F32_MFMA and weight.shape[0] == 32 and weight.shape[-1] <= 32 and feat.is_cuda
                 and (weight.shape[-1] == 32 or not feat.requires_grad)):
-            return _SubMConv3dF32.apply(feat, weight, bias, nbr, rowperm, blocks_fn, walk_fn, has_dup, dup_fn)
+            return _SubMConv3dF32.apply(feat, weight, bias, nbr, rowperm, blocks_fn, walk_fn, has_dup, dup_fn, dbh)
         if weight.shape[0] % 8 == 0 and feat.is_cuda:
-            return _SubMConv3dSplit.apply(feat, weight, bias, nbr, rowperm, blocks_fn, has_dup, dup_fn)
+            return _SubMConv3dSplit.apply(feat, weight, bias, nbr, rowperm, blocks_fn, has_dup, dup_fn, dbh)
         compute_dtype = torch.float32
     return _SubMConv3d.apply(feat, weight, bias, nbr, has_dup, compute_dtype)
 
@@ -575,7 +610,7 @@
 
     def add(self, x, dy, dw, db):
         self.queue.append((x, dy, dw, db))
-        self.bytes += x.numel() * x.element_size() + dy.numel() * dy.element_size()
+        self.bytes += (x.numel() * x.element_size() if x is not None else 0) + dy.numel() * dy.element_size()
         if self.bytes > WGRAD_GROUP_MAX_BYTES:
             q, self.queue, self.bytes = self.queue, [], 0
             nv.linear_wgrad_group(q)
diff --git a/scenesplat_amd/native.py b/scenesplat_amd/native.py
--- a/scenesplat_amd/native.py
+++ b/scenesplat_amd/native.py
@@ -268,7 +268,7 @@
     return torch.zeros(int(numel), dtype=torch.float32, device=device)
 
 
-def subm_conv_wgrad(x, dout, nbr, rowperm, blocks, out=None, nbr_walk=None):
+def subm_conv_wgrad(x, dout, nbr, rowperm, blocks, out=None, nbr_walk=None, dbias=None):
     n, cin = x.shape
     cout = dout.shape[1]
     taps = nbr.shape[0]
@@ -277,14 +277,21 @@
         raise RuntimeError("subm_conv_wgrad: channels must be multiples of 8")
     if rowperm is not None:
         _req(rowperm, torch.int32, "rowperm", (n,))
-    dw = zeros_f32(cout * taps * cin, x.device).view(cout, taps, cin) if out is None else _req(out, torch.float32, "out", (cout, taps, cin))
+    db = None
+    if dbias is True and out is None:
+        buf = zeros_f32(cout * taps * cin + cout, x.device)
+        dw, db = buf[:cout * taps * cin].view(cout, taps, cin), buf[cout * taps * cin:]
+    else:
+        if dbias is not None:
+            db = zeros_f32(cout, x.device) if dbias is True else _req(dbias, torch.float32, "dbias", (cout,))
+        dw = zeros_f32(cout * taps * cin, x.device).view(cout, taps, cin) if out is None else _req(out, torch.float32, "out", (cout, taps, cin))
     cnt, lst = blocks
     _req(cnt, torch.int32, "blk_count", (taps,)); _req(lst, torch.int32, "blk_list", (taps, (n + 63) // 64))
     if nbr_walk is not None:
         _req(nbr_walk, torch.int32, "nbr_walk", (taps, n))
-    check(lib().ss_subm_conv_wgrad_walk(_p(x), _p(dout), _p(nbr), _p(nbr_walk), _p(rowperm), _p(cnt), _p(lst), _p(dw), n, cin, cout, taps,
-                                        _stream()), "ss_subm_conv_wgrad")
-    return dw
+    check(lib().ss_subm_conv_wgrad_bias(_p(x), _p(dout), _p(nbr), _p(nbr_walk), _p(rowperm), _p(cnt), _p(lst), _p(dw), _p(db), n, cin, cout,
+                                        taps, _stream()), "ss_subm_conv_wgrad")
+    return dw if dbias is None else (dw, db)
 
 
 def subm_f32_weight_layout(w, mirror=False):
@@ -344,7 +351,7 @@
     return x
 
 
-def subm_f32_wgrad(x, dout, nbr, rowperm, blocks, cin):
+def subm_f32_wgrad(x, dout, nbr, rowperm, blocks, cin, want_bias=False):
     n, cp = x.shape
     taps = nbr.shape[0]
     _req(x, torch.float32, "x"); _req(dout, torch.float32, "dout", (n, 32)); _req(nbr, torch.int32, "nbr", (taps, n))
@@ -352,17 +359,24 @@
         _req(rowperm, torch.int32, "rowperm", (n,))
     cnt, lst = blocks
     _req(cnt, torch.int32, "blk_count", (taps,)); _req(lst, torch.int32, "blk_list", (taps, (n + 63) // 64))
-    dw = zeros_f32(32 * taps * cin, x.device).view(32, taps, cin)
-    check(lib().ss_subm_f32_wgrad(_p(x), _p(dout), _p(nbr), _p(rowperm), _p(cnt), _p(lst), _p(dw), n, cp, cin, 32, taps, _stream()),
-          "ss_subm_f32_wgrad")
-    return dw
-
-
-def subm_conv_wgrad_pipe(x, dout, nbr, rowperm, blocks):
+    buf = zeros_f32(32 * taps * cin + (32 if want_bias else 0), x.device)
+    dw = buf[:32 * taps * cin].view(32, taps, cin)
+    db = buf[32 * taps * cin:] if want_bias else None
+    check(lib().ss_subm_f32_wgrad_bias(_p(x), _p(dout), _p(nbr), _p(rowperm), _p(cnt), _p(lst), _p(dw), _p(db), n, cp, cin, 32, taps,
+                                       _stream()), "ss_subm_f32_wgrad")
+    return (dw, db) if want_bias else dw
+
+
+def subm_conv_wgrad_pipe(x, dout, nbr, rowperm, blocks, want_bias=False, walk=False):
     n, cin = x.shape
     cout, taps = dout.shape[1], nbr.shape[0]
     dw = torch.zeros((cout, taps, cin), dtype=torch.float32, device=x.device)
     cnt, lst = blocks
+    if want_bias or walk:
+        db = torch.zeros(cout, dtype=torch.float32, device=x.device) if want_bias else None
+        check(lib().ss_subm_conv_wgrad_pipe_bias(_p(x), _p(dout), _p(nbr), _p(rowperm), _p(cnt), _p(lst), _p(dw), _p(db), n, cin, cout,
+                                                 taps, 1 if walk else 0, _stream()), "ss_subm_conv_wgrad_pipe_bias")
+        return (dw, db) if want_bias else dw
     check(lib().ss_subm_conv_wgrad_pipe(_p(x), _p(dout), _p(nbr), _p(rowperm), _p(cnt), _p(lst), _p(dw), n, cin, cout, taps,
                                         _stream()), "ss_subm_conv_wgrad_pipe")
     return dw
@@ -380,14 +394,41 @@
     check(lib().ss_linear_wgrad(_p(x), _p(dy), _p(dw), _p(db), m, k, nout, _stream()), "ss_linear_wgrad")
 
 
+def _bias_only_problem(dy, db, row):
+    m, nout = dy.shape
+    _req(dy, torch.bfloat16, "dy"); _req(db, torch.float32, "db", (nout,))
+    nwg = lib().ss_linear_wgrad_group_plan_bias(m, nout, ctypes.c_void_p(row.ctypes.data)) if dy.data_ptr() % 16 == 0 else 0
+    if nwg <= 0:
+        raise RuntimeError("bias-only weight-gradient problem: needs a 16-byte aligned dy of 8 k <= 4096 columns")
+    row[0], row[1], row[2], row[3], row[4] = 0, dy.data_ptr(), 0, db.data_ptr(), m
+    return nwg
+
+
+def bias_wgrad_into(dy, db):
+    if dy.shape[0] == 0:
+        return
+    desc = np.zeros((1, 8), dtype=np.int64)
+    nwg = _bias_only_problem(dy, db, desc[0])
+    grouped.launch("ss_linear_wgrad_group", desc, grouped.starts([nwg]), dy.device)
+
+
 def linear_wgrad_group(items):
     if not items:
         return
-    dev = items[0][0].device
+    dev = items[0][1].device
     desc = np.zeros((len(items), 8), dtype=np.int64)
     counts = []
-    launch_tiles = sum(lib().ss_linear_wgrad_tiles(x.shape[1], dy.shape[1]) for x, dy, _, _ in items)
+    launch_tiles = sum(lib().ss_linear_wgrad_tiles(x.shape[1], dy.shape[1]) for x, dy, _, _ in items if x is not None)
     for x, dy, dw, db in items:
+        if x is None:
+            j = len(counts)
+            if dy.shape[0] == 0:
+                continue
+            if j >= 128:
+                bias_wgrad_into(dy, db)
+                continue
+            counts.append(_bias_only_problem(dy, db, desc[j]))
+            continue
         _req(x, torch.bfloat16, "x"); _req(dy, torch.bfloat16, "dy", (x.shape[0], dy.shape[1]))
         _req(dw, torch.float32, "dw", (dy.shape[1], x.shape[1]))
         if db is not None:
diff --git a/scenesplat_amd/pointcept_api/ptv3.py b/scenesplat_amd/pointcept_api/ptv3.py
--- a/scenesplat_amd/pointcept_api/ptv3.py
+++ b/scenesplat_amd/pointcept_api/ptv3.py
@@ -1,5 +1,6 @@
 import os
 from functools import partial
+from types import SimpleNamespace
 
 import torch
 import torch.nn as nn
@@ -15,6 +16,7 @@
 RUNTIME = dict(attn_impl=nv.ATTN_SIMT, conv_dtype=None,
                attn_headmajor=os.environ.get("SS_ATTN_HM", "1") != "0",
                param_shadows=os.environ.get("SS_PARAM_SHADOWS", "1") != "0",
+               conv_dbias_hip=os.environ.get("SS_CONV_DBIAS_HIP", "1") != "0",
                fuse_block_tail=os.environ.get("SS_BLOCK_TAIL", "1") != "0")
 
 
@@ -72,7 +74,7 @@
         return SF.subm_conv3d(feat, self.weight, self.bias, level.neighbors(self.kernel_size),
                               level.has_duplicates, cd, level.conv_rowperm(),
                               lambda: level.conv_blocks(self.kernel_size), lambda: level.neighbors_walk(self.kernel_size),
-                              level.dup_runs)
+                              level.dup_runs, dbias_hip=RUNTIME.get("conv_dbias_hip", True) and SF.CONV_DBIAS_HIP)
 
 
 def _lin(mod, x):
@@ -445,6 +447,7 @@
         if ls is None:
             skip = self._modulation_linears()
             ls = [m for m in stage.modules() if isinstance(m, (nn.Linear, nn.LayerNorm)) and id(m) not in skip]
+            ls += [SimpleNamespace(weight=None, bias=m.bias) for m in stage.modules() if isinstance(m, SubMConv3d) and m.bias is not None]
             cache[id(stage)] = ls
         return ls
 
```

New measurement: 2.887 million, median of 4. About the same (+0.2%).
